# alexmeli100/pbrt-rust

Hardware: AMD Instinct MI355X
Metric: Msamples/s (camera rays x spp) at 1920x1080 (higher is better)
Workload: dtype f32

## Files before the change

### pbrt-rust_amd/csrc/dev_light.h

```cpp
#pragma once
#include "dev_scene.h"
#include "dev_sampler.h"
#include "dev_sphere.h"

namespace ptd {

PT_DEV int find_interval_cdf(const float *cdf, int size, float u) {
    int first = 0, len = size;
    while (len > 0) {
        int half = len >> 1, middle = first + half;
        if (cdf[middle] <= u) { first = middle + 1; len -= half + 1; }
        else len = half;
    }
    int r = first - 1;
    return r < 0 ? 0 : (r > size - 2 ? size - 2 : r);
}

struct Dist1D { const float *func; const float *cdf; float func_int; int n; };

PT_DEV int dist_sample_discrete(const Dist1D &d, float u, float &pdf) {
    if (d.n >= 1 && d.n <= 3) {
        const int n = d.n;
        const float c0 = d.cdf[0], c1 = d.cdf[1], c2 = d.cdf[n < 2 ? n : 2], c3 = d.cdf[n < 3 ? n : 3];
        const float f0 = d.func[0], f1 = d.func[n < 2 ? 0 : 1], f2 = d.func[n < 3 ? 0 : 2];
        int first = 0, len = n + 1;
        while (len > 0) {
            const int half = len >> 1, middle = first + half;
            const float cm = middle == 0 ? c0 : middle == 1 ? c1 : middle == 2 ? c2 : c3;
            if (cm <= u) { first = middle + 1; len -= half + 1; }
            else len = half;
        }
        const int r = first - 1;
        const int off = r < 0 ? 0 : (r > n - 1 ? n - 1 : r);
        const float fo = off == 0 ? f0 : off == 1 ? f1 : f2;
        pdf = (d.func_int > 0.0f) ? fo / (d.func_int * (float)n) : 0.0f;
        return off;
    }
    int off = find_interval_cdf(d.cdf, d.n + 1, u);
    pdf = (d.func_int > 0.0f) ? d.func[off] / (d.func_int * (float)d.n) : 0.0f;
    return off;
}
PT_DEV float dist_sample_continuous(const Dist1D &d, float u, float &pdf, int &off) {
    off = find_interval_cdf(d.cdf, d.n + 1, u);
    float du = u - d.cdf[off];
    float diff = d.cdf[off + 1] - d.cdf[off];
    if (diff > 0.0f) du /= diff;
    pdf = (d.func_int > 0.0f) ? d.func[off] / d.func_int : 0.0f;
    return ((float)off + du) / (float)d.n;
}

struct IData { V3 p, p_error, n; };

PT_DEV void spawn_ray(const IData &it, V3 d, V3 &o) { o = offset_ray_origin(it.p, it.p_error, it.n, d); }
PT_DEV void spawn_ray_to(const IData &a, const IData &b, V3 &o, V3 &d) {
    o = offset_ray_origin(a.p, a.p_error, a.n, b.p - a.p);
    V3 t = offset_ray_origin(b.p, b.p_error, b.n, o - b.p);
    d = t - o;
}

PT_DEV RGB env_lookup(const DeviceScene &s, P2 st) {
    int w = (int)s.env_w, h = (int)s.env_h;
    float sf = st.x * (float)w - 0.5f, tf = st.y * (float)h - 0.5f;
    int64_t s0 = f2i_sat(floorf(sf)), t0 = f2i_sat(floorf(tf));
    float ds = sf - (float)s0, dt = tf - (float)t0;
    auto wrap = [](int64_t v, int n) -> int {
        if (v >= -(int64_t)n && v < 2 * (int64_t)n) { int r = (int)v; if (r < 0) r += n; else if (r >= n) r -= n; return r; }
        int64_t r = v % n; if (r < 0) r += n;
        return (int)r;
    };
    const int sa = wrap(s0, w), sb = wrap(s0 + 1, w), ta = wrap(t0, h), tb = wrap(t0 + 1, h);
    auto texel = [&](int si, int ti) -> RGB {
        const float *p = s.env_texels + 3 * ((size_t)ti * w + si);
        return RGB(p[0], p[1], p[2]);
    };
    RGB tmp1 = texel(sb, tb) * (ds * dt);
    RGB tmp2 = texel(sb, ta) * (ds * (1.0f - dt));
    RGB tmp3 = texel(sa, tb) * ((1.0f - ds) * dt);
    RGB tmp4 = texel(sa, ta) * ((1.0f - ds) * (1.0f - dt));
    return tmp4 + tmp3 + tmp2 + tmp1;
}

PT_DEV bool light_is_delta(const PtLight &L) { return L.type == PT_LIGHT_DISTANT || L.type == PT_LIGHT_POINT || L.type == PT_LIGHT_SPOT; }

PT_DEV RGB area_l(const PtLight &L, V3 n, V3 w) {
    if (L.two_sided || dot(n, w) > 0.0f) return RGB(L.L[0], L.L[1], L.L[2]);
    return RGB(0.0f);
}
struct LightTri { V3 p0, p1, p2, n_sample, n_pdf; uint32_t fl, tri; float area, inv_area; RGB Lemit; bool two_sided, degenerate; };
PT_DEV bool load_light_tri(const DeviceScene &s, uint32_t li, LightTri &t, bool for_pdf) {
    const float4 *r = s.light_rec + 6 * (size_t)li;
    const float4 q0 = r[0], q1 = r[1], q2 = r[2];
    t.p0 = V3(q0.x, q0.y, q0.z); t.p1 = V3(q1.x, q1.y, q1.z); t.p2 = V3(q2.x, q2.y, q2.z);
    const uint32_t bits = __float_as_uint(q0.w);
    t.fl = bits & 0xffu; t.degenerate = (bits & 0x200u) != 0u; t.tri = __float_as_uint(q1.w); t.area = q2.w;
    if (for_pdf) { const float4 q5 = r[5]; t.n_pdf = V3(q5.x, q5.y, q5.z); }
    else {
        const float4 q3 = r[3], q4 = r[4];
        t.Lemit = RGB(q3.x, q3.y, q3.z); t.two_sided = __float_as_uint(q3.w) != 0u;
        t.n_sample = V3(q4.x, q4.y, q4.z); t.inv_area = q4.w;
    }
    return (bits & 0x100u) != 0u;
}
PT_DEV RGB area_l(const LightTri &t, V3 n, V3 w) { return (t.two_sided || dot(n, w) > 0.0f) ? t.Lemit : RGB(0.0f); }
PT_DEV M4 ldm4(const float *p) { M4 m; for (int i = 0; i < 16; ++i) m.m[i] = p[i]; return m; }

PT_DEV RGB light_le(const DeviceScene &s, const PtLight &L, V3 ray_d) {
    if (L.type != PT_LIGHT_INFINITE) return RGB(0.0f);
    V3 w = normalize(xf_vector(ldm4(L.world_to_light), ray_d));
    P2 st(spherical_phi(w) * kInv2Pi, spherical_theta(w) * kInvPi);
    return env_lookup(s, st);
}

PT_DEV P2 env_sample_continuous(const DeviceScene &s, P2 u, float &pdf) {
    int nu = 2 * (int)s.env_w, nv = 2 * (int)s.env_h;
    Dist1D marg{s.env_marg_func, s.env_marg_cdf, s.env_marg_int, nv};
    float pdf1, pdf0; int v, dummy;
    float d1 = dist_sample_continuous(marg, u.y, pdf1, v);
    Dist1D cond{s.env_func + (size_t)v * nu, s.env_cdf + (size_t)v * (nu + 1), s.env_func_int[v], nu};
    float d0 = dist_sample_continuous(cond, u.x, pdf0, dummy);
    pdf = pdf0 * pdf1;
    return P2(d0, d1);
}
PT_DEV float env_pdf(const DeviceScene &s, P2 p) {
    int nu = 2 * (int)s.env_w, nv = 2 * (int)s.env_h;
    uint32_t iu = f2u32_sat(p.x * (float)nu); if (iu > (uint32_t)(nu - 1)) iu = nu - 1;
    uint32_t iv = f2u32_sat(p.y * (float)nv); if (iv > (uint32_t)(nv - 1)) iv = nv - 1;
    return s.env_func[(size_t)iv * nu + iu] / s.env_marg_int;
}

PT_DEV IData sphere_sample_interaction(const PtSphere &S, const IData &ref, P2 u, float &pdf) {
    const M4 o2w = ldm4g(S.object_to_world), w2o = ldm4g(S.world_to_object);
    const V3 pcenter = xf_point(o2w, V3(0.0f, 0.0f, 0.0f));
    const V3 porigin = offset_ray_origin(ref.p, ref.p_error, ref.n, pcenter - ref.p);
    IData it;
    if (distance_squared(porigin, pcenter) <= S.radius * S.radius) {
        const float z = 1.0f - 2.0f * u.x;
        const float r = sqrtf(maxf(1.0f - z * z, 0.0f));
        const float phi = 2.0f * kPi * u.y;
        float sn, cs; dm_sincosf(phi, sn, cs);
        V3 pobj = V3(0.0f, 0.0f, 0.0f) + V3(r * cs, r * sn, z) * S.radius;
        it.n = normalize(xf_normal_inv(w2o, pobj));
        if (S.reverse_orientation) it.n = it.n * -1.0f;
        pobj = pobj * (S.radius / length(pobj));
        const V3 perr = vabs(pobj) * gammaf(5);
        it.p = xf_point_abs_err(o2w, pobj, perr, it.p_error);
        pdf = 1.0f / (S.phi_max * S.radius * (S.z_max - S.z_min));
        V3 wi = it.p - ref.p;
        if (length_squared(wi) == 0.0f) pdf = 0.0f;
        else { wi = normalize(wi); pdf *= distance_squared(ref.p, it.p) / abs_dot(it.n, -wi); }
        if (__builtin_isinf(pdf)) pdf = 0.0f;
        return it;
    }
    const float dc = length(ref.p - pcenter);
    const float invdc = 1.0f / dc;
    const V3 wc = (pcenter - ref.p) * invdc; V3 wcx, wcy;
    coordinate_system(wc, wcx, wcy);
    const float sin_thetamax = S.radius * invdc;
    const float sin_thetamax2 = sin_thetamax * sin_thetamax;
    const float inv_sin_thetamax = 1.0f / sin_thetamax;
    const float cos_thetamax = sqrtf(maxf(1.0f - sin_thetamax2, 0.0f));
    float cos_theta = (cos_thetamax - 1.0f) * u.x + 1.0f;
    float sin_theta2 = 1.0f - cos_theta * cos_theta;
    if (sin_thetamax2 < 0.00068523f) { sin_theta2 = sin_thetamax2 * u.x; cos_theta = sqrtf(1.0f - sin_theta2); }
    const float cos_alpha = sin_theta2 * inv_sin_thetamax + cos_theta * sqrtf(maxf(1.0f - sin_theta2 * inv_sin_thetamax * inv_sin_thetamax, 0.0f));
    const float sin_alpha = sqrtf(maxf(1.0f - cos_alpha * cos_alpha, 0.0f));
    const float phi = u.y * 2.0f * kPi;
    float sn, cs; dm_sincosf(phi, sn, cs);
    const V3 nworld = (-wcx) * sin_alpha * cs + (-wcy) * sin_alpha * sn + (-wc) * cos_alpha;
    const V3 pworld = pcenter + V3(nworld.x, nworld.y, nworld.z) * S.radius;
    it.p = pworld; it.p_error = vabs(pworld) * gammaf(5); it.n = V3(0.0f, 0.0f, 0.0f);
    pdf = 1.0f / (2.0f * kPi * (1.0f - cos_thetamax));
    return it;
}

template <bool SPH> PT_DEV RGB light_sample_li(const DeviceScene &s, uint32_t li, const IData &ref, P2 u, V3 &wi, float &pdf, IData &p1) {
    p1.p = V3(); p1.p_error = V3(); p1.n = V3();
    {
        LightTri t;
        if (load_light_tri(s, li, t, false)) {
            const float su0 = sqrtf(u.x);
            const float b0 = 1.0f - su0, b1 = u.y * su0;
            IData it;
            const float b2 = 1.0f - b0 - b1;
            it.p = t.p0 * b0 + t.p1 * b1 + t.p2 * b2;
            it.n = t.n_sample;
            if (t.fl & PT_TRI_HAS_N) {
                const uint32_t i0 = s.indices[3 * t.tri], i1 = s.indices[3 * t.tri + 1], i2 = s.indices[3 * t.tri + 2];
                const V3 ns = ld3(s.N, i0) * b0 + ld3(s.N, i1) * b1 + ld3(s.N, i2) * b2;
                it.n = face_forward(it.n, ns);
            }
            const V3 pabs = vabs(t.p0 * b0) + vabs(t.p1 * b1) + vabs(t.p2 * b2);
            it.p_error = pabs * gammaf(6);
            pdf = t.inv_area;
            V3 w = it.p - ref.p;
            if (length_squared(w) == 0.0f) pdf = 0.0f;
            else {
                w = normalize(w);
                pdf *= distance_squared(ref.p, it.p) / abs_dot(it.n, -w);
                if (__builtin_isinf(pdf)) pdf = 0.0f;
            }
            if (pdf == 0.0f || length_squared(it.p - ref.p) == 0.0f) { pdf = 0.0f; return RGB(0.0f); }
            wi = normalize(it.p - ref.p);
            p1 = it;
            return area_l(t, it.n, -wi);
        }
    }
    const PtLight &L = s.lights[li];
    switch (L.type) {
    case PT_LIGHT_DIFFUSE_AREA: {
        if (SPH && (s.prim_shape[L.prim] >> 30) == PT_SHAPE_SPHERE && s.spheres[s.prim_shape[L.prim] & 0x3fffffffu].kind == PT_QUADRIC_DISK) {
            const PtSphere &S = s.spheres[s.prim_shape[L.prim] & 0x3fffffffu];
            const P2 pd = concentric_sample_disk(u);
            const M4 o2w = ldm4g(S.object_to_world), w2o = ldm4g(S.world_to_object);
            IData it;
            it.n = normalize(xf_normal_inv(w2o, V3(0.0f, 0.0f, 0.1f)));
            if (S.reverse_orientation) it.n = it.n * -1.0f;
            it.p = xf_point_abs_err(o2w, V3(pd.x * S.radius, pd.y * S.radius, S.z_min), V3(0.0f, 0.0f, 0.0f), it.p_error);
            pdf = 1.0f / s.light_area[li];
            V3 w = it.p - ref.p;
            if (length_squared(w) == 0.0f) pdf = 0.0f;
            else {
                w = normalize(w);
                pdf *= distance_squared(ref.p, it.p) / abs_dot(it.n, -w);
                if (__builtin_isinf(pdf)) pdf = 0.0f;
            }
            if (pdf == 0.0f || length_squared(it.p - ref.p) == 0.0f) { pdf = 0.0f; return RGB(0.0f); }
            wi = normalize(it.p - ref.p);
            p1 = it;
            return area_l(L, it.n, -wi);
        }
        if (SPH && (s.prim_shape[L.prim] >> 30) == PT_SHAPE_SPHERE) {
            IData it = sphere_sample_interaction(s.spheres[s.prim_shape[L.prim] & 0x3fffffffu], ref, u, pdf);
            if (pdf == 0.0f || length_squared(it.p - ref.p) == 0.0f) { pdf = 0.0f; return RGB(0.0f); }
            wi = normalize(it.p - ref.p);
            p1 = it;
            return area_l(L, it.n, -wi);
        }
        pdf = 0.0f; return RGB(0.0f);
    }
    case PT_LIGHT_DISTANT: {
        V3 wl(L.dir[0], L.dir[1], L.dir[2]);
        wi = wl; pdf = 1.0f;
        p1.p = ref.p + wl * (2.0f * s.world_radius);
        return RGB(L.L[0], L.L[1], L.L[2]);
    }
    case PT_LIGHT_POINT: {
        V3 pl(L.pos[0], L.pos[1], L.pos[2]);
        wi = normalize(pl - ref.p); pdf = 1.0f;
        p1.p = pl;
        return RGB(L.L[0], L.L[1], L.L[2]) / distance_squared(pl, ref.p);
    }
    case PT_LIGHT_SPOT: {
        V3 pl(L.pos[0], L.pos[1], L.pos[2]);
        wi = normalize(pl - ref.p); pdf = 1.0f;
        p1.p = pl;
        V3 wl = normalize(xf_vector(ldm4(L.world_to_light), -wi));
        float cos_theta = wl.z, fall;
        if (cos_theta < L.cos_total_width) fall = 0.0f;
        else if (cos_theta >= L.cos_falloff_start) fall = 1.0f;
        else { float delta = (cos_theta - L.cos_total_width) / (L.cos_falloff_start - L.cos_total_width); fall = (delta * delta) * (delta * delta); }
        return RGB(L.L[0], L.L[1], L.L[2]) * fall / distance_squared(pl, ref.p);
    }
    case PT_LIGHT_INFINITE: {
        float map_pdf = 0.0f;
        P2 uv = env_sample_continuous(s, u, map_pdf);
        if (map_pdf == 0.0f) { pdf = 0.0f; return RGB(0.0f); }
        float theta = uv.y * kPi, phi = uv.x * 2.0f * kPi;
        float cos_t, sin_t, sin_p, cos_p;
        dm_sincosf(theta, sin_t, cos_t);
        dm_sincosf(phi, sin_p, cos_p);
        V3 v(sin_t * cos_p, sin_t * sin_p, cos_t);
        wi = xf_vector(ldm4(L.light_to_world), v);
        pdf = map_pdf / (2.0f * kPi * kPi * sin_t);
        if (sin_t == 0.0f) pdf = 0.0f;
        p1.p = ref.p + wi * (2.0f * s.world_radius);
        return env_lookup(s, uv);
    }
    default: pdf = 0.0f; return RGB(0.0f);
    }
}

template <bool SPH> PT_DEV float light_pdf_li(const DeviceScene &s, uint32_t li, const IData &ref, V3 wi) {
    {
        LightTri t;
        if (load_light_tri(s, li, t, true)) {
            V3 o; spawn_ray(ref, wi, o);
            float th, b0, b1, b2;
            if (!tri_hit_params(t.p0, t.p1, t.p2, o, wi, PT_INF, th, b0, b1, b2)) return 0.0f;
            if (t.degenerate) return 0.0f;
            const V3 ip = t.p0 * b0 + t.p1 * b1 + t.p2 * b2;
            const V3 in = t.n_pdf;
            float pdf = distance_squared(ref.p, ip) / (dot(in, -wi) * t.area);
            if (__builtin_isinf(pdf)) pdf = 0.0f;
            return pdf;
        }
    }
    const PtLight &L = s.lights[li];
    if (SPH && L.type == PT_LIGHT_DIFFUSE_AREA && (s.prim_shape[L.prim] >> 30) == PT_SHAPE_SPHERE && s.spheres[s.prim_shape[L.prim] & 0x3fffffffu].kind == PT_QUADRIC_DISK) {
        const PtSphere &S = s.spheres[s.prim_shape[L.prim] & 0x3fffffffu];
        V3 o; spawn_ray(ref, wi, o);
        SurfaceInteraction il;
        if (!sphere_fill_interaction(S, o, wi, il, false)) return 0.0f;
        float pdf = distance_squared(ref.p, il.p) / (dot(il.n, -wi) * s.light_area[li]);
        if (__builtin_isinf(pdf)) pdf = 0.0f;
        return pdf;
    }
    if (SPH && L.type == PT_LIGHT_DIFFUSE_AREA && (s.prim_shape[L.prim] >> 30) == PT_SHAPE_SPHERE) {
        const PtSphere &S = s.spheres[s.prim_shape[L.prim] & 0x3fffffffu];
        const V3 pcenter = xf_point(ldm4g(S.object_to_world), V3(0.0f, 0.0f, 0.0f));
        const V3 porigin = offset_ray_origin(ref.p, ref.p_error, ref.n, pcenter - ref.p);
        if (distance_squared(porigin, pcenter) <= S.radius * S.radius) {
            V3 o; spawn_ray(ref, wi, o);
            SurfaceInteraction il;
            if (!sphere_fill_interaction(S, o, wi, il)) return 0.0f;
            float pdf = distance_squared(ref.p, il.p) / (dot(il.n, -wi) * s.light_area[li]);
            if (__builtin_isinf(pdf)) pdf = 0.0f;
            return pdf;
        }
        const float sin_thetamax2 = S.radius * S.radius / distance_squared(ref.p, pcenter);
        const float cos_thetamax = sqrtf(maxf(1.0f - sin_thetamax2, 0.0f));
        return 1.0f / (2.0f * kPi * (1.0f - cos_thetamax));
    }
    if (L.type == PT_LIGHT_DIFFUSE_AREA) return 0.0f;
    if (L.type == PT_LIGHT_INFINITE) {
        V3 w = xf_vector(ldm4(L.world_to_light), wi);
        float theta = spherical_theta(w), phi = spherical_phi(w);
        float sin_t = dm_sinf(theta);
        if (sin_t == 0.0f) return 0.0f;
        return env_pdf(s, P2(phi * kInv2Pi, theta * kInvPi)) / (2.0f * kPi * kPi * sin_t);
    }
    return 0.0f;
}

struct LightGrid {
    int strategy;
    uint32_t nvox[3];
    uint32_t n_lights;
    const float *func;
    const float *cdf;
    const float *func_int;
    const unsigned long long *cell_ptr;
    unsigned long long zero_block;
    uint32_t *missing;
};
PT_DEV size_t light_grid_cell(const LightGrid &g, const DeviceScene &s, V3 p) {
    float o[3] = {p.x - s.wb_min[0], p.y - s.wb_min[1], p.z - s.wb_min[2]};
    uint32_t pi[3];
    for (int i = 0; i < 3; ++i) {
        if (s.wb_max[i] > s.wb_min[i]) o[i] /= s.wb_max[i] - s.wb_min[i];
        const float x = o[i] * (float)g.nvox[i];
        const uint32_t hi = g.nvox[i] - 1u;
        const uint32_t v = (x > 0.0f) ? (uint32_t)(int32_t)fminf(x, 2147483520.0f) : 0u;
        pi[i] = v > hi ? hi : v;
    }
    return ((size_t)pi[2] * g.nvox[1] + pi[1]) * g.nvox[0] + pi[0];
}
PT_DEV Dist1D light_distribution_lookup(const LightGrid &g, const DeviceScene &s, V3 p) {
    size_t cell = 0;
    if (g.strategy == PT_LS_SPATIAL) cell = light_grid_cell(g, s, p);
    if (g.cell_ptr) {
        const unsigned long long b = g.cell_ptr[cell];
        if (b == g.zero_block) atomicAdd(g.missing, 1u);
        const float *blk = reinterpret_cast<const float *>(b);
        Dist1D d{blk + 4, blk + 4 + g.n_lights, blk[0], (int)g.n_lights};
        return d;
    }
    Dist1D d{g.func + cell * g.n_lights, g.cdf + cell * (g.n_lights + 1), g.func_int[cell], (int)g.n_lights};
    return d;
}

}
```

### pbrt-rust_amd/csrc/dev_scene.h

```cpp
#pragma once
#include "dev_math.h"
#include "../../include/mi355pt.h"

namespace ptd {

struct TriPacket {
    float x[3]; uint32_t prim;
    float y[3]; uint32_t shape;
    float z[3]; uint32_t flags;
};
enum { TP_ALPHA = 1u << 7, TP_BOGUS = 1u << 8, TP_SPHERE = 1u << 9, TP_LAST = 1u << 10, TP_INSTANCE = 1u << 11 };
constexpr uint32_t kTpClassShift = 12, kTpClassMask = 15u, kTpMatShift = 16, kTpMatNone = 0xffffu;

struct WideNode {
    float lmin[3]; float lmax0;
    float lmax12[2]; float rmin01[2];
    float rmin2; float rmax[3];
    uint32_t left_ref, right_ref;
    uint32_t meta;
    uint32_t pad;
};
struct QuadNode {
    float lo[3][4];
    float hi[3][4];
    uint32_t ref[4];
    uint32_t meta; uint32_t pad[3];
};
static_assert(sizeof(QuadNode) == 128, "QuadNode is one 128-byte line");
constexpr uint32_t kLeafBit = 0x80000000u;
constexpr uint32_t kRefMask = 0x01ffffffu;
constexpr uint32_t kRefMaskQuad = 0x7fffffffu;

struct DevInstance {
    float world_to_instance[16], instance_to_world[16];
    float root_min[3], root_max[3];
    uint32_t root_ref;
    uint32_t single;
    uint32_t identity;
    uint32_t root_ref4;
};

struct DevGridAux { const float *density; float sigma_t, inv_max_density; };

struct DevBssTable { int n_rho, n_radius; const float *rho_samples, *radius_samples, *profile, *rhoeff, *profile_cdf; };

struct DevImage { uint32_t width, height, n_levels, channels; const float *texels; uint32_t level_offset[16]; };

struct DeviceScene {
    const WideNode *wide; uint32_t n_nodes;
    float root_min[3], root_max[3]; uint32_t root_ref;
    const QuadNode *quad; uint32_t root_ref4; uint32_t leaf_off, pool_quads;
    const TriPacket *leaf; uint32_t n_prims;
    const float *P; const float *N; const float *S; const float *UV;
    const uint32_t *indices; const uint8_t *tri_flags; uint32_t n_triangles;
    const PtSphere *spheres; uint32_t n_spheres;
    const DevInstance *instances; uint32_t n_instances;
    const uint32_t *prim_shape; const uint32_t *prim_material; const uint32_t *prim_light;
    const PtMaterial *materials; uint32_t n_materials;
    const PtLight *lights; uint32_t n_lights;
    const float *light_area;
    const float4 *light_rec;
    const uint32_t *infinite_lights; uint32_t n_infinite;
    const uint8_t *mat_class;
    const DevBssTable *bss_tables; uint32_t n_bss_tables;
    const PtMedium *media; uint32_t n_media;
    uint32_t has_shells;
    const DevGridAux *grid_aux; uint32_t has_grid;
    const uint32_t *prim_med_in; const uint32_t *prim_med_out;
    const PtTexture *textures; uint32_t n_textures; const uint32_t *tex_prog_offset; const uint32_t *tex_prog;
    const DevImage *images; const float *ewa_lut;
    const int32_t *tri_alpha; const int32_t *tri_shadow_alpha;
    uint32_t env_w, env_h; const float *env_texels;
    const float *env_func; const float *env_cdf; const float *env_func_int;
    const float *env_marg_func; const float *env_marg_cdf; float env_marg_int;
    float wb_min[3], wb_max[3];
    float world_radius; float world_center[3];
};

struct Ray { V3 o, d; float t_max; };

struct Hit { uint32_t prim; float t, b0, b1, b2; };

PT_DEV V3 ld3(const float *p, uint32_t i) { return V3(p[3 * i], p[3 * i + 1], p[3 * i + 2]); }

struct TriRay { int kz; float Sx, Sy, Sz; };
PT_DEV TriRay tri_ray_setup(V3 rd) {
    TriRay r;
    r.kz = max_dimension(vabs(rd));
    float dx, dy, dz;
    if (r.kz == 0) { dx = rd.y; dy = rd.z; dz = rd.x; }
    else if (r.kz == 1) { dx = rd.z; dy = rd.x; dz = rd.y; }
    else { dx = rd.x; dy = rd.y; dz = rd.z; }
    r.Sx = -dx / dz; r.Sy = -dy / dz; r.Sz = 1.0f / dz;
    return r;
}
PT_DEV V3 tri_permute(V3 v, int kz) { const bool k0 = kz == 0, k1 = kz == 1; return V3(k0 ? v.y : (k1 ? v.z : v.x), k0 ? v.z : (k1 ? v.x : v.y), k0 ? v.x : (k1 ? v.y : v.z)); }
PT_DEV uint32_t tp_aux(uint32_t w0, uint32_t w1, uint32_t w2, int kz, int axis) {
    const bool k0 = kz == 0, k1 = kz == 1;
    if (axis == 2) return k0 ? w1 : (k1 ? w0 : w2);
    if (axis == 1) return k0 ? w0 : (k1 ? w2 : w1);
    return k0 ? w2 : (k1 ? w1 : w0);
}
PT_DEV bool tri_hit_core(V3 p0t, V3 p1t, V3 p2t, const TriRay &tr, float t_max, float &t, float &b0, float &b1, float &b2) {
    const float Sx = tr.Sx, Sy = tr.Sy, Sz = tr.Sz;
    p0t.x += Sx * p0t.z; p0t.y += Sy * p0t.z;
    p1t.x += Sx * p1t.z; p1t.y += Sy * p1t.z;
    p2t.x += Sx * p2t.z; p2t.y += Sy * p2t.z;
    float e0 = p1t.x * p2t.y - p1t.y * p2t.x;
    float e1 = p2t.x * p0t.y - p2t.y * p0t.x;
    float e2 = p0t.x * p1t.y - p0t.y * p1t.x;
    if (e0 == 0.0f || e1 == 0.0f || e2 == 0.0f) {
        double p2txp1ty = (double)p2t.x * (double)p1t.y, p2typ1tx = (double)p2t.y * (double)p1t.x;
        e0 = (float)(p2typ1tx - p2txp1ty);
        double p0txp2ty = (double)p0t.x * (double)p2t.y, p0typ2tx = (double)p0t.y * (double)p2t.x;
        e1 = (float)(p0typ2tx - p0txp2ty);
        double p1txp0ty = (double)p1t.x * (double)p0t.y, p1typ0tx = (double)p1t.y * (double)p0t.x;
        e2 = (float)(p1typ0tx - p1txp0ty);
    }
    const bool mixed = ((e0 < 0.0f) | (e1 < 0.0f) | (e2 < 0.0f)) & ((e0 > 0.0f) | (e1 > 0.0f) | (e2 > 0.0f));
    float det = e0 + e1 + e2;
    p0t.z *= Sz; p1t.z *= Sz; p2t.z *= Sz;
    float tscaled = e0 * p0t.z + e1 * p1t.z + e2 * p2t.z;
    const float tmd = t_max * det;
    const bool out_neg = (det < 0.0f) & ((tscaled >= 0.0f) | (tscaled < tmd));
    const bool out_pos = (det > 0.0f) & ((tscaled <= 0.0f) | (tscaled >= tmd));
    if (mixed | (det == 0.0f) | out_neg | out_pos) return false;
    float invdet = 1.0f / det;
    b0 = e0 * invdet; b1 = e1 * invdet; b2 = e2 * invdet;
    t = tscaled * invdet;
    float maxzt = max_component(vabs(V3(p0t.z, p1t.z, p2t.z)));
    float deltaz = gammaf(3) * maxzt;
    float maxxt = max_component(vabs(V3(p0t.x, p1t.x, p2t.x)));
    float maxyt = max_component(vabs(V3(p0t.y, p1t.y, p2t.y)));
    float deltax = gammaf(5) * (maxxt + maxzt);
    float deltay = gammaf(5) * (maxyt + maxzt);
    float deltae = 2.0f * (gammaf(2) * maxxt * maxyt + deltay * maxxt + deltax * maxyt);
    float maxe = max_component(vabs(V3(e0, e1, e2)));
    float deltat = 3.0f * (gammaf(3) * maxe * maxzt + deltae * maxzt + deltaz * maxe) * fabsf(invdet);
    if (t <= deltat) return false;
    return true;
}
PT_DEV bool tri_hit_params(V3 p0, V3 p1, V3 p2, V3 ro, const TriRay &tr, float t_max, float &t, float &b0, float &b1, float &b2) {
    return tri_hit_core(tri_permute(p0 - ro, tr.kz), tri_permute(p1 - ro, tr.kz), tri_permute(p2 - ro, tr.kz), tr, t_max, t, b0, b1, b2);
}

PT_DEV bool tri_hit_params(V3 p0, V3 p1, V3 p2, V3 ro, V3 rd, float t_max, float &t, float &b0, float &b1, float &b2) {
    return tri_hit_params(p0, p1, p2, ro, tri_ray_setup(rd), t_max, t, b0, b1, b2);
}

PT_DEV void tri_uvs(const DeviceScene &s, uint32_t tri, uint32_t i0, uint32_t i1, uint32_t i2, P2 uv[3]) {
    if (s.tri_flags[tri] & PT_TRI_HAS_UV) {
        uv[0] = P2(s.UV[2 * i0], s.UV[2 * i0 + 1]); uv[1] = P2(s.UV[2 * i1], s.UV[2 * i1 + 1]); uv[2] = P2(s.UV[2 * i2], s.UV[2 * i2 + 1]);
    } else { uv[0] = P2(0.0f, 0.0f); uv[1] = P2(1.0f, 0.0f); uv[2] = P2(1.0f, 1.0f); }
}
PT_DEV bool tri_partials(V3 p0, V3 p1, V3 p2, const P2 uv[3], V3 &dpdu, V3 &dpdv) {
    float duv02x = uv[0].x - uv[2].x, duv02y = uv[0].y - uv[2].y;
    float duv12x = uv[1].x - uv[2].x, duv12y = uv[1].y - uv[2].y;
    V3 dp02 = p0 - p2, dp12 = p1 - p2;
    float determinant = duv02x * duv12y - duv02y * duv12x;
    bool degenerateuv = fabsf(determinant) < 1.0e-8f;
    dpdu = V3(); dpdv = V3();
    if (!degenerateuv) {
        float invdet = 1.0f / determinant;
        dpdu = (dp02 * duv12y - dp12 * duv02y) * invdet;
        dpdv = (dp02 * -duv12x + dp12 * duv02x) * invdet;
    }
    if (degenerateuv || length_squared(cross(dpdu, dpdv)) == 0.0f) {
        V3 ng = cross(p2 - p0, p1 - p0);
        if (length_squared(ng) == 0.0f) return false;
        coordinate_system(normalize(ng), dpdu, dpdv);
    }
    return true;
}

struct SurfaceInteraction {
    V3 p, p_error, n, wo;
    V3 dpdu;
    V3 sh_n, sh_dpdu;
    V3 dpdv; P2 uv;
    V3 sh_dpdv, sh_dndu, sh_dndv;
    bool has_shape, shape_flip;
    uint32_t prim;
};
PT_DEV void tri_fill_from(const DeviceScene &s, uint32_t tri, uint32_t fl, V3 p0, V3 p1, V3 p2, V3 ray_d, float b0, float b1, float b2, bool with_shape, SurfaceInteraction &si) {
    uint32_t i0 = 0, i1 = 0, i2 = 0;
    if (fl & (PT_TRI_HAS_N | PT_TRI_HAS_S | PT_TRI_HAS_UV)) { i0 = s.indices[3 * tri]; i1 = s.indices[3 * tri + 1]; i2 = s.indices[3 * tri + 2]; }
    P2 uv[3];
    if (fl & PT_TRI_HAS_UV) { uv[0] = P2(s.UV[2 * i0], s.UV[2 * i0 + 1]); uv[1] = P2(s.UV[2 * i1], s.UV[2 * i1 + 1]); uv[2] = P2(s.UV[2 * i2], s.UV[2 * i2 + 1]); }
    else { uv[0] = P2(0.0f, 0.0f); uv[1] = P2(1.0f, 0.0f); uv[2] = P2(1.0f, 1.0f); }
    V3 dpdu, dpdv; tri_partials(p0, p1, p2, uv, dpdu, dpdv);
    V3 dp02 = p0 - p2, dp12 = p1 - p2;
    float xabs = fabsf(b0 * p0.x) + fabsf(b1 * p1.x) + fabsf(b2 * p2.x);
    float yabs = fabsf(b0 * p0.y) + fabsf(b1 * p1.y) + fabsf(b2 * p2.y);
    float zabs = fabsf(b0 * p0.z) + fabsf(b1 * p1.z) + fabsf(b2 * p2.z);
    si.p_error = V3(xabs, yabs, zabs) * gammaf(7);
    si.p = p0 * b0 + p1 * b1 + p2 * b2;
    si.dpdu = dpdu; si.sh_dpdu = dpdu; si.dpdv = dpdv; si.sh_dpdv = dpdv;
    si.sh_dndu = V3(0.0f, 0.0f, 0.0f); si.sh_dndv = V3(0.0f, 0.0f, 0.0f);
    si.uv = P2(uv[0].x * b0 + uv[1].x * b1 + uv[2].x * b2, uv[0].y * b0 + uv[1].y * b1 + uv[2].y * b2);
    bool flip = ((fl & PT_TRI_REVERSE_ORIENTATION) != 0) != ((fl & PT_TRI_SWAPS_HANDEDNESS) != 0);
    si.has_shape = with_shape; si.shape_flip = flip;
    V3 nn = normalize(cross(dp02, dp12));
    si.n = nn; si.sh_n = nn;
    si.wo = -ray_d;
    if (flip) { si.n = -nn; si.sh_n = -nn; }
    if (fl & (PT_TRI_HAS_N | PT_TRI_HAS_S)) {
        V3 ns;
        if (fl & PT_TRI_HAS_N) {
            ns = ld3(s.N, i0) * b0 + ld3(s.N, i1) * b1 + ld3(s.N, i2) * b2;
            if (length_squared(ns) > 0.0f) ns = normalize(ns); else ns = si.n;
        } else ns = si.n;
        V3 ss;
        if (fl & PT_TRI_HAS_S) {
            ss = ld3(s.S, i0) * b0 + ld3(s.S, i1) * b1 + ld3(s.S, i2) * b2;
            if (length_squared(ss) > 0.0f) ss = normalize(ss); else ss = normalize(si.dpdu);
        } else ss = normalize(si.dpdu);
        V3 ts = cross(ss, ns);
        if (length_squared(ts) > 0.0f) { ts = normalize(ts); ss = cross(ts, ns); }
        else coordinate_system(ns, ss, ts);
        if (fl & PT_TRI_HAS_N) {
            const float duv02x = uv[0].x - uv[2].x, duv02y = uv[0].y - uv[2].y, duv12x = uv[1].x - uv[2].x, duv12y = uv[1].y - uv[2].y;
            const V3 n0 = ld3(s.N, i0), n1 = ld3(s.N, i1), n2 = ld3(s.N, i2);
            const V3 dn1 = n0 - n2, dn2 = n1 - n2;
            const float det = duv02x * duv12y - duv02y * duv12x;
            if (fabsf(det) < 1.0e-8f) {
                const V3 dn = cross(n2 - n0, n1 - n0);
                if (length_squared(dn) != 0.0f) coordinate_system(dn, si.sh_dndu, si.sh_dndv);
            } else {
                const float invdet = 1.0f / det;
                si.sh_dndu = (dn1 * duv12y - dn2 * duv02y) * invdet;
                si.sh_dndv = (dn1 * -duv12x + dn2 * duv02x) * invdet;
            }
        }
        if (fl & PT_TRI_REVERSE_ORIENTATION) ts = -ts;
        si.sh_n = normalize(cross(ss, ts));
        if (with_shape) {
            if (flip) si.sh_n = -si.sh_n;
            si.n = face_forward(si.n, si.sh_n);
        }
        si.sh_dpdu = ss; si.sh_dpdv = ts;
    }
}
PT_DEV void tri_fill_interaction(const DeviceScene &s, uint32_t tri, V3 ray_d, float b0, float b1, float b2, bool with_shape, SurfaceInteraction &si) {
    const uint32_t i0 = s.indices[3 * tri], i1 = s.indices[3 * tri + 1], i2 = s.indices[3 * tri + 2];
    tri_fill_from(s, tri, s.tri_flags[tri], ld3(s.P, i0), ld3(s.P, i1), ld3(s.P, i2), ray_d, b0, b1, b2, with_shape, si);
}
PT_DEV float tri_area(V3 p0, V3 p1, V3 p2) { return 0.5f * length(cross(p1 - p0, p2 - p0)); }

PT_DEV bool slab_test(const float bmin[3], const float bmax[3], V3 ro, V3 inv_dir, bool nx, bool ny, bool nz, float ray_tmax) {
    float tmin = ((nx ? bmax[0] : bmin[0]) - ro.x) * inv_dir.x;
    float tmax = ((nx ? bmin[0] : bmax[0]) - ro.x) * inv_dir.x;
    float tymin = ((ny ? bmax[1] : bmin[1]) - ro.y) * inv_dir.y;
    float tymax = ((ny ? bmin[1] : bmax[1]) - ro.y) * inv_dir.y;
    const float k = 1.0f + 2.0f * gammaf(3);
    tmax *= k; tymax *= k;
    if (tmin > tymax || tymin > tmax) return false;
    if (tymin > tmin) tmin = tymin;
    if (tymax < tmax) tmax = tymax;
    float tzmin = ((nz ? bmax[2] : bmin[2]) - ro.z) * inv_dir.z;
    float tzmax = ((nz ? bmin[2] : bmax[2]) - ro.z) * inv_dir.z;
    tzmax *= k;
    if (tmin > tzmax || tzmin > tmax) return false;
    if (tzmin > tmin) tmin = tzmin;
    if (tzmax < tmax) tmax = tzmax;
    return (tmin < ray_tmax) && (tmax > 0.0f);
}
PT_DEV bool slab_geo(const float bmin[3], const float bmax[3], V3 ro, V3 inv_dir, bool nx, bool ny, bool nz, float &tmin_out) {
    float tmin = ((nx ? bmax[0] : bmin[0]) - ro.x) * inv_dir.x;
    float tmax = ((nx ? bmin[0] : bmax[0]) - ro.x) * inv_dir.x;
    const float tymin = ((ny ? bmax[1] : bmin[1]) - ro.y) * inv_dir.y;
    float tymax = ((ny ? bmin[1] : bmax[1]) - ro.y) * inv_dir.y;
    const float tzmin = ((nz ? bmax[2] : bmin[2]) - ro.z) * inv_dir.z;
    float tzmax = ((nz ? bmin[2] : bmax[2]) - ro.z) * inv_dir.z;
    const float k = 1.0f + 2.0f * gammaf(3);
    tmax *= k; tymax *= k; tzmax *= k;
    const bool miss_xy = (tmin > tymax) | (tymin > tmax);
    tmin = (tymin > tmin) ? tymin : tmin;
    tmax = (tymax < tmax) ? tymax : tmax;
    const bool miss_z = (tmin > tzmax) | (tzmin > tmax);
    tmin = (tzmin > tmin) ? tzmin : tmin;
    tmax = (tzmax < tmax) ? tzmax : tmax;
    tmin_out = tmin;
    return !(miss_xy | miss_z) & (tmax > 0.0f);
}

}
```

### pbrt-rust_amd/csrc/kern_decl.h

```cpp
#pragma once
#include "kern_common.h"

template <int ANY, int MODE, bool PROBE, int QUADK> __global__ void k_trace(DeviceScene s, TraceJob job);
template <int MAXL, int MODE, int DIFF> __global__ void k_shade(DeviceScene s, RenderConst rc, SobolTables tabs, LightGrid grid, PathSoA ps, ShadeJob job);
template <bool SPH, bool VOL> __global__ void k_shade_miss(DeviceScene s, RenderConst rc, PathSoA ps, ShadeJob job);
template <bool SPH, bool VOL> __global__ void k_bssrdf(DeviceScene s, RenderConst rc, SobolTables tabs, LightGrid grid, PathSoA ps, BssrdfJob job);
__global__ void k_medium_route(DeviceScene s, RenderConst rc, SobolTables tabs, PathSoA ps, const uint32_t *queue, const uint32_t *count_ptr,
                               uint32_t *class_count, uint32_t *c0, uint32_t *c1, uint32_t *c2, uint32_t *c3, uint32_t *c4, uint32_t *c5, uint32_t *error);
__global__ void k_shade_medium(DeviceScene s, RenderConst rc, SobolTables tabs, LightGrid grid, PathSoA ps, ShadeJob job);
__global__ void k_build_packets(DeviceScene s, const uint32_t *ordered, uint32_t n_refs, TriPacket *out);
__global__ void k_mark_leaf_ends(TriPacket *leaf, const uint32_t *last_index, uint32_t n);
__global__ void k_light_area(DeviceScene s, float *area, float4 *rec);
template <int NQ, int CAP> __global__ void k_route(DeviceScene s, const uint32_t *queue, const uint32_t *count_ptr, PathSoA ps, uint32_t *class_count, RouteJob rj);
__global__ void k_generate(RenderConst rc, SobolTables tabs, PathSoA ps, uint32_t *q_ext, uint32_t *q_ext_count, DevCounters *counters);
__global__ void k_film(RenderConst rc, PathSoA ps, const float *filter_table, float *film_rgbw, DevCounters *counters);
template <bool SPH> __global__ void k_film_final(DeviceScene s, RenderConst rc, PathSoA ps, const float *filter_table, float *film_rgbw, DevCounters *counters);
__global__ void k_film_finish(const float *film_rgbw, float *film_xyzw, uint32_t npix);
__global__ void k_film_resolve(const float4 *film_xyzw, uint32_t n_pixels, float scale, float *rgb, uint8_t *srgb8, int packed);
__global__ void k_film_halves_error(const float4 *film_a, const float4 *film_b, uint32_t width, uint32_t height, uint32_t ntx, float *tile_sum, float *tile_err);
__global__ void k_film_error_reduce(const float *tile_sum, const float *tile_err, uint32_t n_tiles, float n_pixels, float *out);
__global__ void k_tiles_select(RenderConst rc, const float *tile_err, float threshold, const uint32_t *candidates, uint32_t n_candidates, uint32_t *out);
__global__ void k_film_sum(FilmSumArgs a, float4 *dst, int accumulate, size_t n_quads);
__global__ void k_light_grid_contrib(DeviceScene s, uint32_t nvx, uint32_t nvy, uint32_t nvz, float *func, const uint32_t *cells, size_t n_cells, size_t stride);
__global__ void k_light_grid_finish(uint32_t n_lights, size_t ncell, float *func, float *cdf, float *func_int, const uint32_t *cells, size_t stride, unsigned long long *cell_ptr);
template <bool SPH> __global__ void k_light_touch(DeviceScene s, LightGrid g, PathSoA ps, const uint32_t *queue, const uint32_t *count_ptr, uint32_t kind, uint32_t max_depth, uint32_t *req_flag, uint32_t *req_list, uint32_t *req_count);
__global__ void k_halton_samples(SobolTables tabs, HaltonParams hp, uint32_t n, const int32_t *pixel_xy, const uint32_t *sample_num,
                                 uint32_t n_dims, float *out, uint64_t *out_index);
__global__ void k_sobol_samples(SobolTables tabs, SobolParams sp, uint32_t n, const int32_t *pixel_xy, const uint32_t *sample_num,
                                uint32_t n_dims, float *out, uint64_t *out_index);
__global__ void k_camera_rays(RenderConst rc, uint32_t n, const float *cs, float *out_o, float *out_d);
__global__ void k_dist1d_sample(const float *func, const float *cdf, float func_int, int n, int discrete, uint32_t n_u, const float *u, float *out_x, float *out_pdf, int32_t *out_off);
```

### pbrt-rust_amd/csrc/kern_misc.h

```cpp
#pragma once
#include "kern_common.h"
#include "kern_film.h"
__global__ void k_build_packets(DeviceScene s, const uint32_t *ordered, uint32_t n_refs, TriPacket *out) {
    uint32_t i = blockIdx.x * blockDim.x + threadIdx.x;
    if (i >= n_refs) return;
    uint32_t prim = ordered[i];
    TriPacket p;
    if (prim & PT_TOP_INSTANCE) {
        p.x[0] = p.x[1] = p.x[2] = p.y[0] = p.y[1] = p.y[2] = p.z[0] = p.z[1] = p.z[2] = 0.0f;
        p.prim = PT_NONE; p.shape = prim & ~PT_TOP_INSTANCE; p.flags = TP_INSTANCE;
        out[i] = p;
        return;
    }
    uint32_t shape = s.prim_shape[prim];
    p.prim = prim; p.shape = shape; p.flags = 0;
    const uint32_t mat = s.prim_material[prim];
    const uint32_t hi = ((mat == PT_NONE ? 0u : (uint32_t)s.mat_class[mat]) << kTpClassShift) | ((mat == PT_NONE || mat >= kTpMatNone ? kTpMatNone : mat) << kTpMatShift);
    if ((shape >> 30) == PT_SHAPE_TRIANGLE) {
        uint32_t tri = shape & 0x3fffffffu;
        uint32_t i0 = s.indices[3 * tri], i1 = s.indices[3 * tri + 1], i2 = s.indices[3 * tri + 2];
        V3 p0 = ld3(s.P, i0), p1 = ld3(s.P, i1), p2 = ld3(s.P, i2);
        P2 uv[3]; tri_uvs(s, tri, i0, i1, i2, uv);
        V3 dpdu, dpdv;
        bool ok = tri_partials(p0, p1, p2, uv, dpdu, dpdv);
        p.x[0] = p0.x; p.x[1] = p1.x; p.x[2] = p2.x; p.y[0] = p0.y; p.y[1] = p1.y; p.y[2] = p2.y; p.z[0] = p0.z; p.z[1] = p1.z; p.z[2] = p2.z;
        p.flags = (uint32_t)s.tri_flags[tri] | (ok ? 0u : (uint32_t)TP_BOGUS) | hi;
        if ((s.tri_alpha && s.tri_alpha[tri] >= 0) || (s.tri_shadow_alpha && s.tri_shadow_alpha[tri] >= 0)) p.flags |= TP_ALPHA;
    } else {
        p.x[0] = p.x[1] = p.x[2] = p.y[0] = p.y[1] = p.y[2] = p.z[0] = p.z[1] = p.z[2] = 0.0f;
        p.flags = TP_SPHERE | hi;
    }
    out[i] = p;
}

__global__ void k_mark_leaf_ends(TriPacket *leaf, const uint32_t *last_index, uint32_t n) {
    uint32_t i = blockIdx.x * blockDim.x + threadIdx.x;
    if (i < n) leaf[last_index[i]].flags |= TP_LAST;
}

__global__ void k_light_area(DeviceScene s, float *area, float4 *rec) {
    uint32_t i = blockIdx.x * blockDim.x + threadIdx.x;
    if (i >= s.n_lights) return;
    float a = 0.0f;
    const PtLight &L = s.lights[i];
    float4 r0 = make_float4(0.0f, 0.0f, 0.0f, 0.0f), r1 = r0, r2 = r0, r4 = r0, r5 = r0;
    if (L.type == PT_LIGHT_DIFFUSE_AREA) {
        uint32_t shape = s.prim_shape[L.prim];
        if ((shape >> 30) == PT_SHAPE_TRIANGLE) {
            uint32_t tri = shape & 0x3fffffffu;
            const V3 p0 = ld3(s.P, s.indices[3 * tri]), p1 = ld3(s.P, s.indices[3 * tri + 1]), p2 = ld3(s.P, s.indices[3 * tri + 2]);
            a = tri_area(p0, p1, p2);
            const uint32_t fl = s.tri_flags[tri];
            const bool flip = ((fl & PT_TRI_REVERSE_ORIENTATION) != 0) != ((fl & PT_TRI_SWAPS_HANDEDNESS) != 0);
            V3 ns = normalize(cross(p1 - p0, p2 - p0));
            if (!(fl & PT_TRI_HAS_N) && flip) ns = ns * -1.0f;
            V3 np = normalize(cross(p0 - p2, p1 - p2));
            if (flip) np = -np;
            P2 uv[3]; tri_uvs(s, tri, s.indices[3 * tri], s.indices[3 * tri + 1], s.indices[3 * tri + 2], uv);
            V3 dpdu, dpdv;
            const bool degenerate = !tri_partials(p0, p1, p2, uv, dpdu, dpdv);
            r4 = make_float4(ns.x, ns.y, ns.z, 1.0f / a); r5 = make_float4(np.x, np.y, np.z, 0.0f);
            r0 = make_float4(p0.x, p0.y, p0.z, __uint_as_float(fl | 0x100u | (degenerate ? 0x200u : 0u)));
            r1 = make_float4(p1.x, p1.y, p1.z, __uint_as_float(tri)); r2 = make_float4(p2.x, p2.y, p2.z, a);
        } else {
            const PtSphere &S = s.spheres[shape & 0x3fffffffu];
            a = S.kind == PT_QUADRIC_DISK ? S.phi_max * 0.5f * (S.radius * S.radius - S.inner_radius * S.inner_radius)
                                          : S.phi_max * S.radius * (S.z_max - S.z_min);
        }
    }
    area[i] = a;
    float4 *r = rec + 6 * (size_t)i;
    r[0] = r0; r[1] = r1; r[2] = r2; r[3] = make_float4(L.L[0], L.L[1], L.L[2], __uint_as_float(L.two_sided)); r[4] = r4; r[5] = r5;
}
template <int NQ, int CAP>
__global__ __launch_bounds__(256) void k_route(DeviceScene s, const uint32_t *queue, const uint32_t *count_ptr, PathSoA ps, uint32_t *class_count, RouteJob rj) {
    __shared__ LdsQueue<CAP> q[NQ];
#pragma unroll
    for (int k = 0; k < NQ; ++k) lq_init(q[k]);
    __syncthreads();
    const uint32_t count = *count_ptr;
    const uint32_t rounded = (count + 255u) & ~255u;
    for (uint32_t qi = blockIdx.x * blockDim.x + threadIdx.x; qi < rounded; qi += gridDim.x * blockDim.x) {
        const bool valid = qi < count;
        uint32_t pid = 0, cls = (uint32_t)kMissClass;
        if (valid) {
            pid = queue[qi];
            cls = (ps.hit_pflags(pid) >> kTpClassShift) & kTpClassMask;
        }
        const uint32_t slot = (uint32_t)(rj.slot_map >> (4u * cls)) & 15u;
        if (valid && slot == 15u && cls != rj.drop_cls) atomicMax(rj.error, (uint32_t)PT_ERR_UNSUPPORTED);
#pragma unroll
        for (int k = 0; k < NQ; ++k) if ((uint32_t)k < rj.n_slots) lq_push(q[k], pid, valid && slot == (uint32_t)k);
        __syncthreads();
#pragma unroll
        for (int k = 0; k < NQ; ++k) if ((uint32_t)k < rj.n_slots) lq_flush_nosync(q[k], class_count + rj.cls_of_slot[k], rj.buf[k], 256u, false);
        __syncthreads();
    }
#pragma unroll
    for (int k = 0; k < NQ; ++k) if ((uint32_t)k < rj.n_slots) lq_flush_nosync(q[k], class_count + rj.cls_of_slot[k], rj.buf[k], 0u, true);
}
PT_DEV void camera_ray(const RenderConst &rc, float pfx, float pfy, float time_u, P2 plens_u, V3 &o, V3 &d) {
    V3 pcamera = xf_point(rc.raster_to_camera, V3(pfx, pfy, 0.0f));
    V3 ro(0.0f, 0.0f, 0.0f), rd = normalize(pcamera);
    if (rc.lens_radius > 0.0f) {
        P2 dsk = concentric_sample_disk(plens_u);
        float lx = dsk.x * rc.lens_radius, ly = dsk.y * rc.lens_radius;
        float ft = rc.focal_distance / rd.z;
        V3 pfocus = ro + rd * ft;
        ro = V3(lx, ly, 0.0f);
        rd = normalize(pfocus - ro);
    }
    (void)time_u;
    V3 oerr;
    V3 ow = xf_point_err(rc.camera_to_world, ro, oerr);
    V3 dw = xf_vector(rc.camera_to_world, rd);
    float l2 = length_squared(dw);
    if (l2 > 0.0f) { float dt = dot(vabs(dw), oerr) / l2; ow = ow + dw * dt; }
    o = ow; d = dw;
}

constexpr int kGenPlane = 257;
struct GenStage { float4 core[4 * kGenPlane]; float4 ray[2 * kGenPlane]; uint32_t alive[256]; };
PT_DEV void stage_path(GenStage &g, uint32_t t, float pfx, float pfy, V3 o, V3 d, uint64_t index, uint32_t medium) {
    g.core[0 * kGenPlane + t] = make_float4(0.0f, 0.0f, 0.0f, 1.0f);
    g.core[1 * kGenPlane + t] = make_float4(1.0f, 1.0f, 1.0f, __uint_as_float(5u | (PF_CAMERA_RAY << 24)));
    g.core[2 * kGenPlane + t] = make_float4(__uint_as_float((uint32_t)index), __uint_as_float((uint32_t)(index >> 32)), pfx, pfy);
    g.core[3 * kGenPlane + t] = make_float4(__uint_as_float(medium), __uint_as_float(PT_NONE), 0.0f, 0.0f);
    g.ray[0 * kGenPlane + t] = make_float4(o.x, o.y, o.z, d.x); g.ray[1 * kGenPlane + t] = make_float4(d.y, d.z, 0.0f, 0.0f);
}
PT_DEV void flush_paths(const GenStage &g, const PathSoA &ps, uint32_t pid0, uint32_t t) {
    float4 *core = reinterpret_cast<float4 *>(ps.core) + 4 * (size_t)pid0, *ray = reinterpret_cast<float4 *>(ps.ray) + 2 * (size_t)pid0;
#pragma unroll
    for (uint32_t j = 0; j < 4; ++j) { const uint32_t gq = j * 256u + t, p = gq >> 2, q = gq & 3u; if (g.alive[p]) core[gq] = g.core[q * kGenPlane + p]; }
#pragma unroll
    for (uint32_t j = 0; j < 2; ++j) { const uint32_t gq = j * 256u + t, p = gq >> 1, q = gq & 1u; if (g.alive[p]) ray[gq] = g.ray[q * kGenPlane + p]; }
}

__global__ __launch_bounds__(256) void k_generate(RenderConst rc, SobolTables tabs, PathSoA ps, uint32_t *q_ext, uint32_t *q_ext_count, DevCounters *counters) {
    constexpr uint32_t kVdcNibbles = 13;
    __shared__ uint32_t s_nib[kSobolNibbles * 5 * 16];
    __shared__ uint64_t s_vdc[2 * kVdcNibbles * 16];
    __shared__ LdsQueue<1024> s_q;
    __shared__ GenStage s_gen;
    lq_init(s_q);
    const uint32_t m = (uint32_t)rc.sobol.log2_resolution;
    sobol_stage_lds(s_nib, tabs.nib, 5u, threadIdx.x, blockDim.x);
    if (m > 0) for (uint32_t i = threadIdx.x; i < 2 * kVdcNibbles * 16; i += blockDim.x) {
        const uint32_t which = i / (kVdcNibbles * 16), e = i - which * (kVdcNibbles * 16), j = e >> 4, n = e & 15u;
        const uint64_t *col = (which ? tabs.vdc_inv : tabs.vdc) + (m - 1) * 52 + 4 * j;
        uint64_t v = 0;
        for (uint32_t b = 0; b < 4; ++b) if (n & (1u << b)) v ^= col[b];
        s_vdc[i] = v;
    }
    __syncthreads();
    const uint32_t total = rc.n_pix_slots * rc.s_count;
    const uint32_t stride = gridDim.x * blockDim.x;
    const uint32_t rounded = (total + 255u) & ~255u;
    unsigned long long n_alive = 0;
    for (uint32_t pid = blockIdx.x * blockDim.x + threadIdx.x; pid < rounded; pid += stride) {
        bool alive = false;
        if (pid < total) {
            const uint32_t slot = pid % rc.n_pix_slots, sl = pid / rc.n_pix_slots;
            int32_t px, py;
            if (slot_to_pixel(rc, slot, px, py)) {
                const uint64_t sample = rc.s_begin + sl;
                if (rc.halton.enabled) {
                    const uint64_t index = halton_index_for_sample(rc.halton, px, py, sample);
                    const float fx = halton_sample_dimension(tabs, rc.halton, index, 0u), fy = halton_sample_dimension(tabs, rc.halton, index, 1u);
                    const float pfx = (float)px + fx, pfy = (float)py + fy;
                    const float tm = halton_sample_dimension(tabs, rc.halton, index, 2u);
                    const P2 pl(halton_sample_dimension(tabs, rc.halton, index, 3u), halton_sample_dimension(tabs, rc.halton, index, 4u));
                    V3 o, d;
                    camera_ray(rc, pfx, pfy, tm, pl, o, d);
                    stage_path(s_gen, threadIdx.x, pfx, pfy, o, d, index, rc.volpath ? rc.camera_medium : PT_NONE);
                    alive = true;
                } else {
                uint64_t index = 0;
                if (m != 0) {
                    index = sample << (m << 1);
                    uint64_t delta = 0;
                    for (uint64_t f = sample, j = 0; f != 0; f >>= 4, ++j) delta ^= s_vdc[j * 16 + (f & 15u)];
                    uint64_t b = ((uint64_t)((uint32_t)(px - rc.sobol.sb_min[0]) << m) | (uint64_t)(uint32_t)(py - rc.sobol.sb_min[1])) ^ delta;
                    for (uint32_t j = 0; b != 0; b >>= 4, ++j) index ^= s_vdc[kVdcNibbles * 16 + j * 16 + (b & 15u)];
                }
                const uint32_t v0 = sobol_bits_nib(s_nib, 5u * 16u, tabs.m32, index), v1 = sobol_bits_nib(s_nib + 16, 5u * 16u, tabs.m32 + 52, index), v2 = sobol_bits_nib(s_nib + 32, 5u * 16u, tabs.m32 + 104, index),
                               v3 = sobol_bits_nib(s_nib + 48, 5u * 16u, tabs.m32 + 156, index), v4 = sobol_bits_nib(s_nib + 64, 5u * 16u, tabs.m32 + 208, index);
                float fx = sobol_to_float(v0) * (float)rc.sobol.resolution + (float)rc.sobol.sb_min[0];
                fx = clampf(fx - (float)px, 0.0f, kOneMinusEps);
                float fy = sobol_to_float(v1) * (float)rc.sobol.resolution + (float)rc.sobol.sb_min[1];
                fy = clampf(fy - (float)py, 0.0f, kOneMinusEps);
                const float pfx = (float)px + fx, pfy = (float)py + fy;
                V3 o, d;
                camera_ray(rc, pfx, pfy, sobol_to_float(v2), P2(sobol_to_float(v3), sobol_to_float(v4)), o, d);
                stage_path(s_gen, threadIdx.x, pfx, pfy, o, d, index, rc.volpath ? rc.camera_medium : PT_NONE);
                alive = true;
                }
            }
        }
        s_gen.alive[threadIdx.x] = alive ? 1u : 0u;
        __syncthreads();
        flush_paths(s_gen, ps, pid - threadIdx.x, threadIdx.x);
        lq_push(s_q, pid, alive);
        lq_sync_flush(s_q, q_ext_count, q_ext, 256u, false);
        n_alive += alive ? 1ull : 0ull;
    }
    lq_sync_flush(s_q, q_ext_count, q_ext, 0u, true);
    counter_add(&counters->camera_rays, n_alive);
}
__global__ __launch_bounds__(256) void k_film(RenderConst rc, PathSoA ps, const float *filter_table, float *film_rgbw, DevCounters *counters) {
    film_slot(rc, ps, filter_table, film_rgbw, counters, [](uint32_t, RGB &) {});
}

__global__ void k_film_finish(const float *film_rgbw, float *film_xyzw, uint32_t npix) {
    uint32_t i = blockIdx.x * blockDim.x + threadIdx.x;
    if (i >= npix) return;
    float rgb[3] = {film_rgbw[4 * i], film_rgbw[4 * i + 1], film_rgbw[4 * i + 2]}, xyz[3];
    rgb_to_xyz(rgb, xyz);
    film_xyzw[4 * i] += xyz[0]; film_xyzw[4 * i + 1] += xyz[1]; film_xyzw[4 * i + 2] += xyz[2]; film_xyzw[4 * i + 3] += film_rgbw[4 * i + 3];
}
__global__ void k_film_sum(FilmSumArgs a, float4 *dst, int accumulate, size_t n_quads) {
    const size_t i = (size_t)blockIdx.x * blockDim.x + threadIdx.x;
    if (i >= n_quads) return;
    float4 s = a.src[0][i];
    for (uint32_t k = 1; k < a.n; ++k) { const float4 b = a.src[k][i]; s = make_float4(s.x + b.x, s.y + b.y, s.z + b.z, s.w + b.w); }
    if (accumulate) { const float4 d = dst[i]; s = make_float4(d.x + s.x, d.y + s.y, d.z + s.z, d.w + s.w); }
    dst[i] = s;
}

__global__ __launch_bounds__(256) void k_light_grid_contrib(DeviceScene s, uint32_t nvx, uint32_t nvy, uint32_t nvz, float *func, const uint32_t *cells, size_t n_cells, size_t stride) {
    const size_t gid = (size_t)blockIdx.x * blockDim.x + threadIdx.x;
    const size_t ncell = cells ? n_cells : (size_t)nvx * nvy * nvz;
    if (gid >= ncell * s.n_lights) return;
    const uint32_t j = (uint32_t)(gid % s.n_lights);
    const size_t slot = gid / s.n_lights;
    const size_t cell = cells ? (size_t)cells[slot] : slot;
    const uint32_t pi0 = (uint32_t)(cell % nvx), pi1 = (uint32_t)((cell / nvx) % nvy), pi2 = (uint32_t)(cell / ((size_t)nvx * nvy));
    V3 p0((float)pi0 / (float)nvx, (float)pi1 / (float)nvy, (float)pi2 / (float)nvz);
    V3 p1((float)(pi0 + 1) / (float)nvx, (float)(pi1 + 1) / (float)nvy, (float)(pi2 + 1) / (float)nvz);
    V3 a(lerpf(p0.x, s.wb_min[0], s.wb_max[0]), lerpf(p0.y, s.wb_min[1], s.wb_max[1]), lerpf(p0.z, s.wb_min[2], s.wb_max[2]));
    V3 b(lerpf(p1.x, s.wb_min[0], s.wb_max[0]), lerpf(p1.y, s.wb_min[1], s.wb_max[1]), lerpf(p1.z, s.wb_min[2], s.wb_max[2]));
    V3 vmin(minf(a.x, b.x), minf(a.y, b.y), minf(a.z, b.z)), vmax(maxf(a.x, b.x), maxf(a.y, b.y), maxf(a.z, b.z));
    float contrib = 0.0f;
    for (uint32_t i = 0; i < 128; ++i) {
        V3 u3(radical_inverse(0, i), radical_inverse(1, i), radical_inverse(2, i));
        IData intr;
        intr.p = V3(lerpf(u3.x, vmin.x, vmax.x), lerpf(u3.y, vmin.y, vmax.y), lerpf(u3.z, vmin.z, vmax.z));
        P2 u(radical_inverse(3, i), radical_inverse(4, i));
        float pdf = 0.0f; V3 wi; IData vis;
        RGB Li = light_sample_li<true>(s, j, intr, u, wi, pdf, vis);
        if (pdf > 0.0f) contrib += Li.y() / pdf;
    }
    func[cells ? slot * stride + 4 + j : gid] = contrib;
}
__global__ __launch_bounds__(256) void k_light_grid_finish(uint32_t n_lights, size_t ncell, float *func, float *cdf, float *func_int, const uint32_t *cells, size_t stride, unsigned long long *cell_ptr) {
    const size_t cell = (size_t)blockIdx.x * blockDim.x + threadIdx.x;
    if (cell >= ncell) return;
    float *f = cells ? func + cell * stride + 4 : func + cell * n_lights, *c = cells ? f + n_lights : cdf + cell * (n_lights + 1);
    float sum = 0.0f;
    for (uint32_t j = 0; j < n_lights; ++j) sum += f[j];
    const float avg = sum / (128.0f * (float)n_lights);
    const float min_contrib = (avg > 0.0f) ? 0.001f * avg : 1.0f;
    for (uint32_t j = 0; j < n_lights; ++j) f[j] = maxf(f[j], min_contrib);
    c[0] = 0.0f;
    for (uint32_t i = 1; i < n_lights + 1; ++i) c[i] = c[i - 1] + f[i - 1] / (float)n_lights;
    const float fi = c[n_lights];
    if (fi == 0.0f) { for (uint32_t i = 1; i < n_lights + 1; ++i) c[i] = (float)i / (float)n_lights; }
    else { for (uint32_t i = 1; i < n_lights + 1; ++i) c[i] /= fi; }
    if (cells) { func[cell * stride] = fi; __threadfence(); cell_ptr[cells[cell]] = (unsigned long long)(func + cell * stride); }
    else func_int[cell] = fi;
}

template <bool SPH>
__global__ __launch_bounds__(256) void k_light_touch(DeviceScene s, LightGrid g, PathSoA ps, const uint32_t *queue, const uint32_t *count_ptr, uint32_t kind, uint32_t max_depth,
                                                     uint32_t *req_flag, uint32_t *req_list, uint32_t *req_count) {
    const uint32_t count = *count_ptr;
    for (uint32_t qi = blockIdx.x * blockDim.x + threadIdx.x; qi < count; qi += gridDim.x * blockDim.x) {
        const uint32_t pid = queue[qi];
        const uint32_t meta = ps.meta(pid);
        if ((meta >> 24) & PF_DEAD) continue;
        if (kind != 2u && ((meta >> 16) & 0xffu) >= max_depth) continue;
        const V3 ro(ps.ox(pid), ps.oy(pid), ps.oz(pid)), rd(ps.dx(pid), ps.dy(pid), ps.dz(pid));
        V3 p;
        if (kind == 1u) p = ro + rd * ps.hit_t(pid);
        else {
            if (ps.hit_prim(pid) == PT_NONE) continue;
            SurfaceInteraction si;
            fill_hit_pkt<SPH>(s, ps.hit_pkt(pid), SPH ? ps.hit_inst(pid) : PT_NONE, ro, rd, ps.hit_b0(pid), ps.hit_b1(pid), ps.hit_b2(pid), si);
            p = si.p;
        }
        const size_t cell = light_grid_cell(g, s, p);
        if (g.cell_ptr[cell] == g.zero_block && atomicExch(&req_flag[cell], 1u) == 0u) req_list[atomicAdd(req_count, 1u)] = (uint32_t)cell;
    }
}
__global__ void k_halton_samples(SobolTables tabs, HaltonParams hp, uint32_t n, const int32_t *pixel_xy, const uint32_t *sample_num,
                                 uint32_t n_dims, float *out, uint64_t *out_index) {
    uint32_t i = blockIdx.x * blockDim.x + threadIdx.x;
    if (i >= n) return;
    const uint64_t index = halton_index_for_sample(hp, pixel_xy[2 * i], pixel_xy[2 * i + 1], sample_num[i]);
    if (out_index) out_index[i] = index;
    for (uint32_t d = 0; d < n_dims; ++d) out[(size_t)i * n_dims + d] = halton_sample_dimension(tabs, hp, index, d);
}

__global__ __launch_bounds__(256) void k_sobol_samples(SobolTables tabs, SobolParams sp, uint32_t n, const int32_t *pixel_xy, const uint32_t *sample_num,
                                                       uint32_t n_dims, float *out, uint64_t *out_index) {
    constexpr uint32_t LDS_DIMS = 56u;
    __shared__ uint32_t s_sobol[LDS_DIMS * kSobolNibWords];
    sobol_stage_lds(s_sobol, tabs.nib, LDS_DIMS, threadIdx.x, blockDim.x);
    __syncthreads();
    uint32_t i = blockIdx.x * blockDim.x + threadIdx.x;
    if (i >= n) return;
    int32_t px = pixel_xy[2 * i], py = pixel_xy[2 * i + 1];
    uint64_t index = sobol_interval_to_index(tabs, (uint32_t)sp.log2_resolution, sample_num[i], (uint32_t)(px - sp.sb_min[0]), (uint32_t)(py - sp.sb_min[1]));
    if (out_index) out_index[i] = index;
    for (uint32_t d = 0; d < 2 && d < n_dims; ++d) out[(size_t)i * n_dims + d] = sobol_pixel_dim(tabs.m32, sp, index, (int)d, d == 0 ? px : py);
    Sampler smp; smp.index = index; smp.m32 = tabs.m32; smp.nib = tabs.nib; smp.lds = s_sobol; smp.lds_dims = LDS_DIMS; smp.overflow = false; smp.halton = false;
    smp.prime = tabs.prime; smp.prime_sum = tabs.prime_sum; smp.perm = tabs.perm;
    for (uint32_t d = 2; d < n_dims;) {
        smp.dim = d;
        smp.load_window();
        for (uint32_t k = 0; k < 8 && d < n_dims; ++k, ++d) out[(size_t)i * n_dims + d] = smp.get_1d();
    }
}
__global__ void k_camera_rays(RenderConst rc, uint32_t n, const float *cs, float *out_o, float *out_d) {
    uint32_t i = blockIdx.x * blockDim.x + threadIdx.x;
    if (i >= n) return;
    V3 o, d;
    camera_ray(rc, cs[5 * i], cs[5 * i + 1], cs[5 * i + 2], P2(cs[5 * i + 3], cs[5 * i + 4]), o, d);
    out_o[3 * i] = o.x; out_o[3 * i + 1] = o.y; out_o[3 * i + 2] = o.z;
    out_d[3 * i] = d.x; out_d[3 * i + 1] = d.y; out_d[3 * i + 2] = d.z;
}
__global__ void k_dist1d_sample(const float *func, const float *cdf, float func_int, int n, int discrete, uint32_t n_u, const float *u, float *out_x, float *out_pdf, int32_t *out_off) {
    uint32_t i = blockIdx.x * blockDim.x + threadIdx.x;
    if (i >= n_u) return;
    Dist1D d{func, cdf, func_int, n};
    float pdf = 0.0f; int off = 0; float x = 0.0f;
    if (discrete) off = dist_sample_discrete(d, u[i], pdf);
    else x = dist_sample_continuous(d, u[i], pdf, off);
    out_x[i] = x; out_pdf[i] = pdf; out_off[i] = off;
}
```

### pbrt-rust_amd/csrc/kern_shade_common.h

```cpp
#pragma once
#include "kern_common.h"

#ifdef PT_REGION_PROFILE
struct Prof { long long *t; int *r; unsigned long long *acc; };
#define PT_PROF_BEGIN __shared__ long long s_pt[4]; __shared__ int s_pr[4]; __shared__ unsigned long long s_pacc[64]; \
    if (threadIdx.x < 64) s_pacc[threadIdx.x] = 0; \
    if (threadIdx.x < 4) { s_pt[threadIdx.x] = clock64(); s_pr[threadIdx.x] = 15; } \
    Prof prof{s_pt, s_pr, s_pacc};
#define PT_PROF_END(counters) do { PT_T(14); __syncthreads(); \
    if (threadIdx.x < 16) atomicAdd(&(counters)->regions[threadIdx.x], prof.acc[threadIdx.x] + prof.acc[16 + threadIdx.x] + prof.acc[32 + threadIdx.x] + prof.acc[48 + threadIdx.x]); } while (0)
#define PT_T(k) do { if ((int)__lane_id() == __ffsll((unsigned long long)__ballot(1)) - 1) { const long long _n = clock64(); const int _w = threadIdx.x >> 6; \
    prof.acc[_w * 16 + prof.r[_w]] += (unsigned long long)(_n - prof.t[_w]); prof.t[_w] = _n; prof.r[_w] = (k); } } while (0)
#define PT_PROF_ARG , Prof prof
#define PT_PROF_PASS , prof
#else
#define PT_T(k) do {} while (0)
#define PT_PROF_BEGIN
#define PT_PROF_END(counters) do {} while (0)
#define PT_PROF_ARG
#define PT_PROF_PASS
#endif

template <bool SPH, bool VOL = false, bool EARLY = false> PT_DEV void resolve_pending(const DeviceScene &s, const PathSoA &ps, uint32_t pid, uint32_t &flags, RGB &L,
                                                unsigned long long &zero_num, uint32_t &n_assert, unsigned long long &n_bytes PT_PROF_ARG, Sampler *smp = nullptr) {
    if (!(flags & (PF_PEND_SHADOW | PF_PEND_MIS))) return;
    PT_T(1);
    const float4 *nq = reinterpret_cast<const float4 *>(ps.nee) + 4 * (size_t)pid;
    const float4 n1 = nq[1], n2 = nq[2], n3 = nq[3];
    float4 e0 = make_float4(0.0f, 0.0f, 0.0f, 0.0f), e1 = e0, e2 = e0, e3 = e0;
    if constexpr (EARLY) {
        if (flags & PF_PEND_MIS) { const float4 *mq = reinterpret_cast<const float4 *>(ps.mis) + 4 * (size_t)pid; e0 = mq[0]; e1 = mq[1]; e2 = mq[2]; e3 = mq[3]; }
        asm volatile("" :: "v"(n1.x), "v"(n2.x), "v"(n3.x), "v"(e0.x), "v"(e1.x), "v"(e2.x), "v"(e3.x));
    }
    n_bytes += 48 + ((flags & PF_PEND_MIS) ? 64 : 0);
    RGB Ld(0.0f);
    const uint32_t li = __float_as_uint(n1.w);
    if ((flags & PF_PEND_SHADOW) && (VOL ? __float_as_uint(n1.z) == PT_NONE : __float_as_uint(n1.z) == 0u)) {
        RGB A(n2.x, n2.y, n2.z);
        if (VOL) {
            const uint32_t sm = __float_as_uint(n3.w);
            if (sm != PT_NONE && s.media[sm].type == PT_MEDIUM_GRID) {
                const float4 n0 = nq[0];
                if (smp) A = A * grid_tr(s.media[sm], s.grid_aux[sm], V3(n0.x, n0.y, n0.z), V3(n0.w, n1.x, n1.y), 1.0f - kShadowEps, *smp);
                else A = RGB(0.0f);
            }
        }
        Ld = Ld + A;
    }
    if (flags & PF_PEND_MIS) {
        const float4 *mq = reinterpret_cast<const float4 *>(ps.mis) + 4 * (size_t)pid;
        const float4 m0 = EARLY ? e0 : mq[0], m1 = EARLY ? e1 : mq[1], m2 = EARLY ? e2 : mq[2], m3 = EARLY ? e3 : mq[3];
        const PtLight &Lt = s.lights[li];
        V3 wi(m0.w, m1.x, m1.y);
        RGB lrad(0.0f);
        const uint32_t mp = __float_as_uint(m2.x);
        if (mp != PT_NONE) {
            if (s.prim_light[mp] == li) {
                SurfaceInteraction lsi;
                fill_hit<SPH>(s, mp, PT_NONE, V3(m0.x, m0.y, m0.z), wi, m2.y, m2.z, m2.w, lsi);
                lrad = area_l(Lt, lsi.n, -wi);
            }
        } else { PT_T(2); lrad = light_le(s, Lt, wi); PT_T(1); }
        RGB Tr(1.0f);
        bool tr_done = false;
        if (VOL) {
            const uint32_t mm = ps.mis_medium(pid);
            if (mm != PT_NONE && s.media[mm].type == PT_MEDIUM_GRID) {
                Tr = smp ? RGB(grid_tr(s.media[mm], s.grid_aux[mm], V3(m0.x, m0.y, m0.z), wi, mp != PT_NONE ? m3.w : PT_INF, *smp)) : RGB(0.0f);
                tr_done = true;
            }
        }
        if (!lrad.is_black()) {
            RGB f(m3.x, m3.y, m3.z);
            if (VOL && !tr_done) {
                const uint32_t mm = ps.mis_medium(pid);
                if (mm != PT_NONE) Tr = Tr * medium_tr(s.media[mm], mp != PT_NONE ? m3.w : PT_INF, wi);
            }
            Ld = Ld + f * lrad * Tr * m1.z / m1.w;
        }
    }
    RGB nb(n3.x, n3.y, n3.z);
    RGB Ldb = nb * (Ld / n2.w);
    if (!VOL && Ldb.is_black() && !(flags & PF_NEE_UNCOUNTED)) zero_num++;
    if (!VOL && !(flags & PF_NEE_UNCOUNTED) && !(Ldb.y() >= 0.0f)) n_assert++;
    L = L + Ldb;
    flags &= ~(PF_PEND_SHADOW | PF_PEND_MIS | PF_NEE_UNCOUNTED);
}

template <bool SPH> PT_DEV bool vol_chain_step(const DeviceScene &s, const PathSoA &ps, uint32_t pid, uint32_t flags, Sampler &smp, bool &push_shadow, bool &push_mis,
                                              unsigned long long &n_bytes) {
    float4 *nq = reinterpret_cast<float4 *>(ps.nee) + 4 * (size_t)pid;
    float4 *mq = reinterpret_cast<float4 *>(ps.mis) + 4 * (size_t)pid;
    float4 *xq = reinterpret_cast<float4 *>(ps.ext) + 8 * (size_t)pid;
    if ((flags & PF_PEND_SHADOW) && __float_as_uint(nq[1].z) != 1u) {
        const float4 n0 = nq[0], n1 = nq[1], n2 = nq[2], n3 = nq[3], h0 = xq[4], h1 = xq[5];
        n_bytes += 64 + 32;
        const uint32_t prim = __float_as_uint(h0.x), sm = __float_as_uint(n3.w);
        const bool hit = prim != PT_NONE;
        const V3 so(n0.x, n0.y, n0.z), sd(n0.w, n1.x, n1.y);
        RGB A(n2.x, n2.y, n2.z);
        bool ended = true;
        if (hit && s.prim_material[prim] != PT_NONE) A = RGB(0.0f);
        else {
            if (sm != PT_NONE) {
                const float t_seg = hit ? h1.y : 1.0f - kShadowEps;
                A = A * (s.media[sm].type == PT_MEDIUM_GRID ? RGB(grid_tr(s.media[sm], s.grid_aux[sm], so, sd, t_seg, smp)) : medium_tr(s.media[sm], t_seg, sd));
            }
            if (hit) {
                SurfaceInteraction hs;
                fill_hit_pkt<SPH>(s, __float_as_uint(h1.z), SPH ? __float_as_uint(h1.x) : PT_NONE, so, sd, h0.y, h0.z, h0.w, hs);
                IData a; a.p = hs.p; a.p_error = hs.p_error; a.n = hs.n;
                IData b; { const float4 x0 = xq[0], x1 = xq[1], x2 = xq[2]; b.p = V3(x0.x, x0.y, x0.z); b.p_error = V3(x1.x, x1.y, x1.z); b.n = V3(x2.x, x2.y, x2.z); }
                V3 o2, d2; spawn_ray_to(a, b, o2, d2);
                const uint32_t sm2 = medium_toward(surface_iface(s, prim, sm), hs.n, d2);
                nq[0] = make_float4(o2.x, o2.y, o2.z, d2.x); nq[1] = make_float4(d2.y, d2.z, 0.0f, n1.w); nq[3] = make_float4(n3.x, n3.y, n3.z, __uint_as_float(sm2));
                push_shadow = true; ended = false; n_bytes += 48 + 4;
            }
        }
        nq[2] = make_float4(A.r, A.g, A.b, n2.w);
        if (!ended) return true;
        nq[1] = make_float4(n1.x, n1.y, __uint_as_float(1u), n1.w);
    }
    if (flags & PF_PEND_MIS) {
        const float4 m0 = mq[0], m1 = mq[1], m3 = mq[3], h0 = xq[6], h1 = xq[7];
        n_bytes += 64 + 32;
        const uint32_t prim = __float_as_uint(h0.x), mm = ps.mis_medium(pid);
        const bool hit = prim != PT_NONE;
        const V3 mo(m0.x, m0.y, m0.z), wi(m0.w, m1.x, m1.y);
        RGB f(m3.x, m3.y, m3.z);
        if (mm != PT_NONE) f = f * (s.media[mm].type == PT_MEDIUM_GRID ? RGB(grid_tr(s.media[mm], s.grid_aux[mm], mo, wi, hit ? h1.y : PT_INF, smp)) : medium_tr(s.media[mm], hit ? h1.y : PT_INF, wi));
        if (hit && s.prim_material[prim] == PT_NONE) {
            SurfaceInteraction hs;
            fill_hit_pkt<SPH>(s, __float_as_uint(h1.z), SPH ? __float_as_uint(h1.x) : PT_NONE, mo, wi, h0.y, h0.z, h0.w, hs);
            IData a; a.p = hs.p; a.p_error = hs.p_error; a.n = hs.n;
            V3 o2; spawn_ray(a, wi, o2);
            ps.mis_medium(pid) = medium_toward(surface_iface(s, prim, mm), hs.n, wi);
            mq[0] = make_float4(o2.x, o2.y, o2.z, wi.x); mq[3] = make_float4(f.r, f.g, f.b, m3.w);
            push_mis = true; n_bytes += 32 + 4;
            return true;
        }
        mq[2] = h0; mq[3] = make_float4(f.r, f.g, f.b, hit ? h1.y : 0.0f);
        ps.mis_medium(pid) = PT_NONE;
    }
    if (flags & PF_PEND_SHADOW) {
        const float4 n1 = nq[1], n3 = nq[3];
        nq[1] = make_float4(n1.x, n1.y, __uint_as_float(PT_NONE), n1.w); nq[3] = make_float4(n3.x, n3.y, n3.z, __uint_as_float(PT_NONE));
    }
    return false;
}


template <int QCAP, bool PROBE, bool SELF> struct VertexQueues {
    LdsQueue<QCAP> ext, res, sh, mis;
    LdsQueue<PROBE ? QCAP : 1> probe;
    LdsQueue<SELF ? QCAP : 1> self;
    PT_DEV void init() { lq_init(ext); lq_init(res); lq_init(sh); lq_init(mis); lq_init(probe); lq_init(self); }
    template <class Job> PT_DEV void push(const Job &job, uint32_t pid, bool to_ext, bool to_resolve, bool to_shadow, bool to_mis, bool to_self = false, bool to_probe = false) {
        lq_push(ext, pid, to_ext);
        lq_push(res, pid, to_resolve && job.shade_next0 != nullptr);
        lq_push(sh, pid, to_shadow);
        lq_push(mis, pid, to_mis);
        if constexpr (PROBE) if (job.probe_next) lq_push(probe, pid, to_probe);
        if constexpr (SELF) lq_push(self, pid, to_self);
    }
    template <class Job> PT_DEV void flush(const Job &job, uint32_t reserve, bool force) {
        __syncthreads();
        lq_flush_nosync(ext, job.ext_next_count, job.ext_next, reserve, force);
        lq_flush_nosync(res, job.shade_next0_count, job.shade_next0, reserve, force);
        lq_flush_nosync(sh, job.shadow_count, job.shadow, reserve, force);
        lq_flush_nosync(mis, job.mis_count, job.mis, reserve, force);
        if constexpr (PROBE) if (job.probe_next) lq_flush_nosync(probe, job.probe_next_count, job.probe_next, reserve, force);
        if constexpr (SELF) lq_flush_nosync(self, job.self_next_count, job.self_next, reserve, force);
        __syncthreads();
    }
};

PT_DEV bool russian_roulette(const RenderConst &rc, Sampler &smp, RGB &beta, float etascale, uint32_t bounces, uint32_t &n_assert) {
    const RGB rrbeta = beta * etascale;
    if (rrbeta.max_component_value() < rc.rr_threshold && bounces > 3) {
        const float q = maxf(1.0f - rrbeta.max_component_value(), 0.05f);
        if (smp.get_1d() < q) return true;
        beta = beta / (1.0f - q); if (__builtin_isinf(beta.y())) n_assert++;
    }
    return false;
}

PT_DEV uint32_t vertex_meta(const Sampler &smp, uint32_t bounces, uint32_t flags, uint32_t *error) {
    if (smp.overflow) atomicMax(error, (uint32_t)PT_ERR_SOBOL_DIMENSIONS);
    return (smp.dim & 0xffffu) | ((bounces & 0xffu) << 16) | (flags << 24);
}
PT_DEV void store_vertex(const PathSoA &ps, uint32_t pid, RGB L, RGB beta, const Sampler &smp, uint32_t bounces, uint32_t flags, uint32_t *error) {
    const uint32_t meta = vertex_meta(smp, bounces, flags, error);
    ps.L_r(pid) = L.r; ps.L_g(pid) = L.g; ps.L_b(pid) = L.b;
    ps.beta_r(pid) = beta.r; ps.beta_g(pid) = beta.g; ps.beta_b(pid) = beta.b;
    ps.meta(pid) = meta;
}

PT_DEV void add_escaped_le(const DeviceScene &s, V3 rd, RGB beta, RGB &L) {
    for (uint32_t k = 0; k < s.n_infinite; ++k) L = L + light_le(s, s.lights[s.infinite_lights[k]], rd) * beta;
}

PT_DEV void hist_init(uint32_t *s_hist) { if (threadIdx.x < 16) s_hist[threadIdx.x] = 0; }
PT_DEV void hist_add(uint32_t *s_hist, uint32_t bounces) { atomicAdd(&s_hist[bounces > 15u ? 15u : bounces], 1u); }
PT_DEV void vertex_epilogue(const uint32_t *s_hist, DevCounters *c, unsigned long long *items, unsigned long long *bytes, unsigned long long n_valid, unsigned long long n_bytes,
                            uint32_t n_assert) {
    if (threadIdx.x < 16 && s_hist[threadIdx.x]) atomicAdd(&c->path_len[threadIdx.x], (unsigned long long)s_hist[threadIdx.x]);
    counter_add(&c->ref_asserts, (unsigned long long)n_assert);
    counter_add(&c->stages, n_valid);
    counter_add(items, n_valid);
    counter_add(bytes, n_bytes);
}

template <bool SPH, class B, bool VOL = false, bool MEDIUM = false>
PT_DEV bool nee_vertex(const DeviceScene &s, const LightGrid &grid, const PathSoA &ps, uint32_t pid, Sampler &smp,
                                          const SurfaceInteraction &si, const IData &it, const B &bsdf, RGB beta, uint32_t &flags,
                                          bool &push_shadow, bool &push_mis, unsigned long long &n_bytes PT_PROF_ARG, MedIface mif = MedIface{PT_NONE, PT_NONE}) {
    bool nee_pending = false;
    if (s.n_lights > 0) {
        PT_T(5);
        Dist1D distrib = light_distribution_lookup(grid, s, si.p);
        float choice_pdf = 0.0f;
        const uint32_t li = (uint32_t)dist_sample_discrete(distrib, smp.get_1d(), choice_pdf);
        if (choice_pdf != 0.0f) {
            const P2 ulight = smp.get_2d();
            const P2 uscatt = smp.get_2d();
            const int bf = BSDF_ALL & ~BSDF_SPECULAR;
            V3 wi; float lightpdf = 0.0f, scattpdf = 0.0f; IData p1;
            RGB A(0.0f); V3 sh_o(0.0f, 0.0f, 0.0f), sh_d(0.0f, 0.0f, 0.0f);
            uint32_t sh_medium = PT_NONE;
            PT_T(6);
            RGB Li = light_sample_li<SPH>(s, li, it, ulight, wi, lightpdf, p1);
            PT_T(7);
            const bool delta = light_is_delta(s.lights[li]);
            if (lightpdf > 0.0f && !Li.is_black()) {
                RGB f = bsdf.f_pdf(si.wo, wi, bf, scattpdf);
                if (!MEDIUM) f = f * abs_dot(wi, si.sh_n);
                if (!f.is_black()) {
                    V3 so, sd; spawn_ray_to(it, p1, so, sd);
                    if (VOL) {
                        const uint32_t sm = medium_toward(mif, it.n, sd);
                        if (s.has_shells) {
                            sh_medium = sm;
                            float4 *xq = reinterpret_cast<float4 *>(ps.ext) + 8 * (size_t)pid;
                            xq[0] = make_float4(p1.p.x, p1.p.y, p1.p.z, 0.0f); xq[1] = make_float4(p1.p_error.x, p1.p_error.y, p1.p_error.z, 0.0f); xq[2] = make_float4(p1.n.x, p1.n.y, p1.n.z, 0.0f);
                            n_bytes += 48;
                        }
                        else if (sm != PT_NONE && s.media[sm].type == PT_MEDIUM_GRID) sh_medium = sm;
                        else if (sm != PT_NONE) Li = Li * medium_tr(s.media[sm], 1.0f - kShadowEps, sd);
                    }
                    A = delta ? f * Li / lightpdf : f * Li * power_heuristic(lightpdf, scattpdf) / lightpdf;
                    sh_o = so; sh_d = sd;
                    flags |= PF_PEND_SHADOW; push_shadow = true; nee_pending = true; n_bytes += 16 + 4;
                }
            }
            if (!delta) {
                PT_T(8);
                int sampled_type = 0;
                RGB f = bsdf.sample_f(si.wo, wi, uscatt, scattpdf, bf, sampled_type);
                if (!MEDIUM) f = f * abs_dot(wi, si.sh_n);
                const bool sampled_specular = (sampled_type & BSDF_SPECULAR) != 0;
                if (!f.is_black() && scattpdf > 0.0f) {
                    float weight = 1.0f;
                    bool skip = false;
                    if (!sampled_specular) {
                        PT_T(9);
                        lightpdf = light_pdf_li<SPH>(s, li, it, wi);
                        PT_T(8);
                        if (lightpdf == 0.0f) skip = true;
                        else weight = power_heuristic(scattpdf, lightpdf);
                    }
                    if (!skip) {
                        V3 mo; spawn_ray(it, wi, mo);
                        float4 *mq = reinterpret_cast<float4 *>(ps.mis) + 4 * (size_t)pid;
                        mq[0] = make_float4(mo.x, mo.y, mo.z, wi.x); mq[1] = make_float4(wi.y, wi.z, weight, scattpdf); mq[3] = make_float4(f.r, f.g, f.b, 0.0f);
                        if (VOL) ps.mis_medium(pid) = medium_toward(mif, it.n, wi);
                        flags |= PF_PEND_MIS; push_mis = true; nee_pending = true; n_bytes += 48 + 4;
                    }
                }
            }
            if (nee_pending) {
                float4 *nq = reinterpret_cast<float4 *>(ps.nee) + 4 * (size_t)pid;
                if (flags & PF_PEND_SHADOW) nq[0] = make_float4(sh_o.x, sh_o.y, sh_o.z, sh_d.x);
                nq[1] = make_float4(sh_d.y, sh_d.z, 0.0f, __uint_as_float(li)); nq[2] = make_float4(A.r, A.g, A.b, choice_pdf); nq[3] = make_float4(beta.r, beta.g, beta.b, __uint_as_float(sh_medium));
                n_bytes += 48;
            }
        }
    }
    return nee_pending;
}

struct TexMatEval {
    const DeviceScene &s; const TexCtx &c;
    struct Plain {
        const DeviceScene &s; TexCtx c;
        PT_DEV bool bound(const PtMaterial &m, int slot) const { return m.tex[slot] >= 0; }
        PT_DEV RGB spec(const PtMaterial &m, int slot, const float *field) const { return m.tex[slot] >= 0 ? tex_eval(s, m.tex[slot], c) : RGB(field[0], field[1], field[2]); }
        PT_DEV float flt(const PtMaterial &m, int slot, float field) const { return m.tex[slot] >= 0 ? tex_eval(s, m.tex[slot], c).r : field; }
    };
    PT_DEV Plain plain() const { Plain q{s, c}; q.c.dpdx = V3(0.0f, 0.0f, 0.0f); q.c.dpdy = V3(0.0f, 0.0f, 0.0f); q.c.dudx = q.c.dvdx = q.c.dudy = q.c.dvdy = 0.0f; return q; }
    PT_DEV bool bound(const PtMaterial &m, int slot) const { return m.tex[slot] >= 0; }
    PT_DEV RGB spec(const PtMaterial &m, int slot, const float *field) const { return m.tex[slot] >= 0 ? tex_eval(s, m.tex[slot], c) : RGB(field[0], field[1], field[2]); }
    PT_DEV float flt(const PtMaterial &m, int slot, float field) const { return m.tex[slot] >= 0 ? tex_eval(s, m.tex[slot], c).r : field; }
};
PT_DEV RayDiff camera_ray_differentials(const RenderConst &rc, float pfx, float pfy, P2 plens_u, V3 ray_o, V3 ray_d) {
    const V3 pcamera = xf_point(rc.raster_to_camera, V3(pfx, pfy, 0.0f));
    const V3 dxc(rc.dx_camera[0], rc.dx_camera[1], rc.dx_camera[2]), dyc(rc.dy_camera[0], rc.dy_camera[1], rc.dy_camera[2]);
    RayDiff d; d.has = true;
    if (rc.lens_radius > 0.0f) {
        const P2 dk = concentric_sample_disk(plens_u);
        const float lx = dk.x * rc.lens_radius, ly = dk.y * rc.lens_radius;
        const V3 dx = normalize(pcamera + dxc);
        float ft = rc.focal_distance / dx.z;
        V3 pfocus = V3(0.0f, 0.0f, 0.0f) + (dx * ft);
        d.rx_o = V3(lx, ly, 0.0f); d.rx_d = normalize(pfocus - d.rx_o);
        const V3 dy = normalize(pcamera + dyc);
        ft = rc.focal_distance / dy.z;
        pfocus = V3(0.0f, 0.0f, 0.0f) + (dy * ft);
        d.ry_o = V3(lx, ly, 0.0f); d.ry_d = normalize(pfocus - d.ry_o);
    } else {
        d.rx_o = V3(0.0f, 0.0f, 0.0f); d.ry_o = V3(0.0f, 0.0f, 0.0f);
        d.rx_d = normalize(pcamera + dxc); d.ry_d = normalize(pcamera + dyc);
    }
    d.rx_o = xf_point(rc.camera_to_world, d.rx_o); d.ry_o = xf_point(rc.camera_to_world, d.ry_o);
    d.rx_d = xf_vector(rc.camera_to_world, d.rx_d); d.ry_d = xf_vector(rc.camera_to_world, d.ry_d);
    const float sc = rc.inv_sqrt_spp;
    d.rx_o = ray_o + (d.rx_o - ray_o) * sc; d.ry_o = ray_o + (d.ry_o - ray_o) * sc;
    d.rx_d = ray_d + (d.rx_d - ray_d) * sc; d.ry_d = ray_d + (d.ry_d - ray_d) * sc;
    return d;
}
```

### pbrt-rust_amd/csrc/scene_create.hip

```cpp
#include "host_common.h"

#include <memory>

namespace {
PtStatus hlbvh_builder(const std::vector<pth::PrimBound> &pb, uint32_t maxp, std::vector<PtBVHNode> &nodes, std::vector<uint32_t> &ordered, std::string &msg) {
    const char *text = "HLBVH build failed";
    if (!pth::build_hlbvh_gpu(pb, maxp, nodes, ordered, &text)) return PT_OK;
    msg = text;
    return PT_ERR_HIP;
}
struct Uploader {
    pt_scene *sc; int st = PT_OK;
    template <class T> void operator()(const T **field, const T *src, size_t count) { if (!st) st = sc->upload(field, src, count); }
    template <class T> void operator()(const T **field, const std::vector<T> &v) { (*this)(field, v.data(), v.size()); }
};
}

extern "C" {

int pt_scene_create(const PtSceneDesc *d, pt_scene **out) {
    if (!d || !out) return fail(PT_ERR_INVALID_ARG, "null argument");
    std::string msg;
    int st = plan_validate(*d, msg);
    if (st) return fail(st, msg);
    if ((st = ensure_device())) return st;
    ScenePlan plan;
    if ((st = plan_build(*d, PlanOptions{g_shade_specialise, g_test_pool_pad_records}, d->split_method == PT_SPLIT_HLBVH ? AccelBuilder(hlbvh_builder) : AccelBuilder(sah_builder), plan, msg))) return fail(st, msg);
    for (const std::string &w : plan.warnings) fprintf(stderr, "mi355pt: %s\n", w.c_str());

    std::unique_ptr<pt_scene, void (*)(pt_scene *)> owner(new pt_scene(), pt_scene_destroy);
    pt_scene *sc = owner.get();
    DeviceScene &ds = sc->ds;
    sc->device = g_device;
    sc->nodes = std::move(plan.nodes); sc->ordered = std::move(plan.ordered);
    sc->exact_walk_only = plan.exact_walk_only; sc->quad_walk_only = plan.quad_walk_only; sc->pool_big = plan.pool_big;
    std::copy(plan.class_used, plan.class_used + kNumClasses, sc->class_used);
    sc->has_null_material = plan.has_null_material; sc->has_bssrdf = plan.has_bssrdf;
    sc->n_lights = d->n_lights;
    if (d->n_lights) sc->host_lights.assign(d->lights, d->lights + d->n_lights);
    if (d->env_texels) { sc->env_w = d->env_width; sc->env_h = d->env_height; for (int k = 0; k < 3; ++k) sc->env_texel0[k] = d->env_power_lookup[k]; }

    Uploader up{sc};
    up(&ds.wide, plan.wide); ds.root_ref = plan.root_ref; ds.root_ref4 = plan.root_ref4; ds.n_nodes = (uint32_t)sc->nodes.size();
    for (int k = 0; k < 3; ++k) { ds.root_min[k] = sc->nodes[0].bmin[k]; ds.root_max[k] = sc->nodes[0].bmax[k]; }
    up(&ds.instances, plan.instances); ds.n_instances = (uint32_t)plan.instances.size();
    up(&ds.P, d->P, 3 * (size_t)d->n_vertices);
    if (d->N) up(&ds.N, d->N, 3 * (size_t)d->n_vertices);
    if (d->S) up(&ds.S, d->S, 3 * (size_t)d->n_vertices);
    if (d->UV) up(&ds.UV, d->UV, 2 * (size_t)d->n_vertices);
    up(&ds.indices, d->indices, 3 * (size_t)d->n_triangles); ds.n_triangles = d->n_triangles;
    {
        std::vector<uint8_t> fl(d->n_triangles, 0);
        if (d->tri_flags) fl.assign(d->tri_flags, d->tri_flags + d->n_triangles);
        for (auto &f : fl) { if (!d->N) f &= ~PT_TRI_HAS_N; if (!d->S) f &= ~PT_TRI_HAS_S; if (!d->UV) f &= ~PT_TRI_HAS_UV; }
        up(&ds.tri_flags, fl);
    }
    up(&ds.prim_shape, d->prim_shape, d->n_prims); up(&ds.prim_material, d->prim_material, d->n_prims); up(&ds.prim_light, d->prim_light, d->n_prims);
    ds.n_prims = d->n_prims;
    up(&ds.materials, d->materials, d->n_materials); ds.n_materials = d->n_materials;
    if (d->n_media && d->media) {
        up(&ds.media, d->media, d->n_media); ds.n_media = d->n_media;
        for (uint32_t i = 0; i < d->n_media; ++i)
            if (d->media[i].type == PT_MEDIUM_GRID) up(&plan.grid_aux[i].density, d->media[i].density, (size_t)d->media[i].nx * d->media[i].ny * d->media[i].nz);
        up(&ds.grid_aux, plan.grid_aux); ds.has_grid = plan.has_grid ? 1u : 0u;
        if (d->prim_medium_inside && d->prim_medium_outside) { up(&ds.prim_med_in, d->prim_medium_inside, d->n_prims); up(&ds.prim_med_out, d->prim_medium_outside, d->n_prims); }
    }
    ds.has_shells = sc->has_null_material ? 1u : 0u;
    up(&ds.spheres, d->spheres, d->n_spheres); ds.n_spheres = d->n_spheres;
    up(&ds.lights, d->lights, d->n_lights); ds.n_lights = d->n_lights;
    up(&ds.mat_class, plan.mat_class);
    {
        std::vector<DevBssTable> bt(d->n_bssrdf_tables);
        for (uint32_t i = 0; i < d->n_bssrdf_tables; ++i) {
            const PtBSSRDFTable &t = d->bssrdf_tables[i];
            bt[i].n_rho = (int)t.n_rho; bt[i].n_radius = (int)t.n_radius;
            if (!t.rho_samples || !t.radius_samples || !t.profile || !t.rhoeff || !t.profile_cdf) continue;
            up(&bt[i].rho_samples, t.rho_samples, t.n_rho); up(&bt[i].radius_samples, t.radius_samples, t.n_radius);
            up(&bt[i].profile, t.profile, (size_t)t.n_rho * t.n_radius);
            up(&bt[i].rhoeff, t.rhoeff, t.n_rho);
            up(&bt[i].profile_cdf, t.profile_cdf, (size_t)t.n_rho * t.n_radius);
        }
        up(&ds.bss_tables, bt); ds.n_bss_tables = d->n_bssrdf_tables;
    }
    if (d->n_textures) {
        up(&ds.textures, d->textures, d->n_textures); ds.n_textures = d->n_textures;
        up(&ds.tex_prog_offset, plan.tex_prog_offset); up(&ds.tex_prog, plan.tex_prog);
        for (uint32_t i = 0; i < d->n_images; ++i) {
            const PtImage &im = d->images[i];
            if (!im.texels || im.n_levels == 0 || im.n_levels > 16) continue;
            const uint32_t last = im.n_levels - 1;
            up(&plan.images[i].texels, im.texels, plan.images[i].level_offset[last] + (size_t)std::max(1u, im.width >> last) * std::max(1u, im.height >> last) * im.channels);
        }
        up(&ds.images, plan.images);
        if (d->ewa_weight_lut) up(&ds.ewa_lut, d->ewa_weight_lut, 128);
        auto any_mask = [&](const int32_t *a) { if (!a) return false; for (uint32_t i = 0; i < d->n_triangles; ++i) if (a[i] >= 0) return true; return false; };
        if (any_mask(d->tri_alpha)) up(&ds.tri_alpha, d->tri_alpha, d->n_triangles);
        if (any_mask(d->tri_shadow_alpha)) up(&ds.tri_shadow_alpha, d->tri_shadow_alpha, d->n_triangles);
    }
    up(&ds.infinite_lights, plan.infinite_lights); ds.n_infinite = (uint32_t)plan.infinite_lights.size();
    if (d->env_texels) {
        ds.env_w = d->env_width; ds.env_h = d->env_height;
        up(&ds.env_texels, d->env_texels, 3 * (size_t)ds.env_w * ds.env_h);
        up(&ds.env_func, d->env_importance, 4 * (size_t)ds.env_w * ds.env_h); up(&ds.env_cdf, plan.env_cdf); up(&ds.env_func_int, plan.env_func_int);
        up(&ds.env_marg_func, plan.env_func_int); up(&ds.env_marg_cdf, plan.env_marg_cdf); ds.env_marg_int = plan.env_marg_int;
    }
    for (int k = 0; k < 3; ++k) { ds.wb_min[k] = plan.wb_min[k]; ds.wb_max[k] = plan.wb_max[k]; ds.world_center[k] = plan.world_center[k]; }
    ds.world_radius = plan.world_radius;
    const uint32_t *d_ordered = nullptr, *d_last = nullptr;
    up(&d_ordered, plan.packet_refs);
    if (up.st) return up.st;

    const uint32_t n_packets = (uint32_t)plan.packet_refs.size(), n_leaves = (uint32_t)plan.leaf_last.size();
    uint8_t *pool = nullptr; float *area = nullptr; float4 *lrec = nullptr;
    if ((st = sc->dalloc(&pool, plan.pool_bytes))) return st;
    if (plan.pad_bytes && hipMemset(pool, 0, plan.pad_bytes) != hipSuccess) return fail(PT_ERR_HIP, "memset of the pool pad");
    if (hipMemcpy(pool + plan.pad_bytes, plan.quad.data(), plan.quad_bytes - plan.pad_bytes, hipMemcpyHostToDevice) != hipSuccess) return fail(PT_ERR_HIP, "upload of the four-wide records");
    TriPacket *leaf = reinterpret_cast<TriPacket *>(pool + plan.quad_bytes);
    ds.quad = reinterpret_cast<const QuadNode *>(pool); ds.leaf_off = (uint32_t)(plan.quad_bytes / 16); ds.pool_quads = (uint32_t)(plan.pool_bytes / 16);
    if (hipMemset(leaf, 0, ((size_t)n_packets + 2) * sizeof(TriPacket)) != hipSuccess) return fail(PT_ERR_HIP, "memset");
    if ((st = sc->dalloc(&area, std::max<uint32_t>(1, d->n_lights)))) return st;
    if ((st = sc->dalloc(&lrec, 6 * (size_t)std::max<uint32_t>(1, d->n_lights)))) return st;
    up(&d_last, plan.leaf_last);
    if (up.st) return up.st;
    hipLaunchKernelGGL(k_build_packets, dim3((n_packets + 255) / 256), dim3(256), 0, 0, ds, d_ordered, n_packets, leaf);
    ds.leaf = leaf;
    hipLaunchKernelGGL(k_mark_leaf_ends, dim3((n_leaves + 255) / 256), dim3(256), 0, 0, leaf, d_last, n_leaves);
    if (d->n_lights) hipLaunchKernelGGL(k_light_area, dim3((d->n_lights + 255) / 256), dim3(256), 0, 0, ds, area, lrec);
    ds.light_area = area; ds.light_rec = lrec;
    if (hipDeviceSynchronize() != hipSuccess || hipGetLastError() != hipSuccess) return fail(PT_ERR_HIP, "scene preparation kernels failed");
    *out = owner.release();
    return PT_OK;
}

void pt_scene_destroy(pt_scene *sc) {
    if (!sc) return;
    if (sc->device != g_device) bind_device(sc->device);
    for (void *p : sc->allocs) hipFree(p);
    if (sc->slab) hipFree(sc->slab);
    if (sc->qbuf) hipFree(sc->qbuf);
    if (sc->bss_slab) hipFree(sc->bss_slab);
    if (sc->ext_slab) hipFree(sc->ext_slab);
    if (sc->film_rgbw) hipFree(sc->film_rgbw);
    if (sc->tile_list) hipFree(sc->tile_list);
    sc->drop_timings();
    for (auto e : sc->event_pool) hipEventDestroy(e);
    if (sc->stream) hipStreamDestroy(sc->stream);
    delete sc;
}

int pt_scene_bvh_info(const pt_scene *sc, uint32_t *n_nodes, uint32_t *n_prims) {
    if (!sc || !n_nodes || !n_prims) return fail(PT_ERR_INVALID_ARG, "null argument");
    *n_nodes = (uint32_t)sc->nodes.size(); *n_prims = (uint32_t)sc->ordered.size();
    return PT_OK;
}
int pt_scene_bvh_read(const pt_scene *sc, PtBVHNode *nodes, uint32_t *ordered) {
    if (!sc || !nodes || !ordered) return fail(PT_ERR_INVALID_ARG, "null argument");
    std::memcpy(nodes, sc->nodes.data(), sc->nodes.size() * sizeof(PtBVHNode));
    std::memcpy(ordered, sc->ordered.data(), sc->ordered.size() * 4);
    return PT_OK;
}

}
```

### pbrt-rust_amd/csrc/scene_plan.h

```cpp
#pragma once
#include <functional>
#include <string>
#include <vector>
#include "kernels.h"
#include "host_bvh.h"

namespace pth {
using namespace ptd;

uint8_t material_class(const PtMaterial &m, bool specialise, bool untextured);
void dist1d(const std::vector<float> &func, std::vector<float> &cdf, float &func_int);
PrimBound transform_bounds(const float m[16], const float lo[3], const float hi[3]);

struct PlanOptions {
    bool shade_specialise = true;
    uint32_t pool_pad_records = 0;
};
using AccelBuilder = std::function<PtStatus(const std::vector<PrimBound> &prims, uint32_t max_node_prims, std::vector<PtBVHNode> &nodes, std::vector<uint32_t> &ordered, std::string &msg)>;
PtStatus sah_builder(const std::vector<PrimBound> &prims, uint32_t max_node_prims, std::vector<PtBVHNode> &nodes, std::vector<uint32_t> &ordered, std::string &msg);

struct ScenePlan {
    std::vector<PtBVHNode> nodes;
    std::vector<uint32_t> ordered;
    bool exact_walk_only = false, quad_walk_only = false, pool_big = false;
    std::vector<WideNode> wide;
    std::vector<QuadNode> quad;
    uint32_t root_ref = 0, root_ref4 = 0;
    std::vector<uint32_t> packet_refs;
    std::vector<uint32_t> leaf_last;
    std::vector<DevInstance> instances;
    size_t pad_bytes = 0, quad_bytes = 0, pool_bytes = 0;
    std::vector<uint8_t> mat_class;
    bool class_used[kNumClasses] = {true, false, false, false, true, false, false, false, false, false, false};
    bool has_null_material = false, has_bssrdf = false;
    std::vector<uint32_t> infinite_lights;
    std::vector<uint32_t> tex_prog_offset, tex_prog;
    std::vector<DevImage> images;
    std::vector<float> env_cdf, env_func_int, env_marg_cdf; float env_marg_int = 0.0f;
    std::vector<DevGridAux> grid_aux; bool has_grid = false;
    float wb_min[3] = {0, 0, 0}, wb_max[3] = {0, 0, 0}, world_center[3] = {0, 0, 0}, world_radius = 0.0f;
    std::vector<std::string> warnings;
};

PtStatus plan_validate(const PtSceneDesc &d, std::string &msg);
PtStatus plan_build(const PtSceneDesc &d, const PlanOptions &opt, const AccelBuilder &build, ScenePlan &plan, std::string &msg);

}
```

### pbrt-rust_amd/csrc/scene_plan.hip

```cpp
#include <algorithm>
#include <cmath>
#include <cstring>
#include <limits>
#include "scene_plan.h"
#include "dev_bsdf.h"
#include "dev_texture.h"

namespace pth {

uint8_t material_class(const PtMaterial &m, bool specialise, bool untextured) {
    auto textured = [&](int slot) { return m.tex[slot] >= 0; };
    auto black = [](const float c[3]) { return !(c[0] > 0.0f) && !(c[1] > 0.0f) && !(c[2] > 0.0f); };
    switch (m.type) {
    case PT_MAT_MATTE: return 0;
    case PT_MAT_MIRROR: return (uint8_t)kSpecClass;
    case PT_MAT_METAL: return specialise ? (uint8_t)kMetalClass : 1;
    case PT_MAT_SUBSTRATE: return 1;
    case PT_MAT_GLASS:
        if (textured(PT_MP_U_ROUGHNESS) || textured(PT_MP_V_ROUGHNESS)) return 2;
        return (m.u_roughness == 0.0f && m.v_roughness == 0.0f) ? (uint8_t)kSpecClass : 2;
    case PT_MAT_PLASTIC: return specialise ? (uint8_t)kPlasticClass : 2;
    case PT_MAT_UBER: {
        const bool opaque = !textured(PT_MP_OPACITY) && m.opacity[0] >= 1.0f && m.opacity[1] >= 1.0f && m.opacity[2] >= 1.0f;
        const bool no_spec = !textured(PT_MP_KR) && !textured(PT_MP_KT) && black(m.kr) && black(m.kt);
        if (opaque && no_spec) return specialise ? (uint8_t)kPlasticClass : 2;
        return specialise ? (uint8_t)kUberClass : 3;
    }
    case PT_MAT_SUBSURFACE:
        if (specialise && untextured && m.u_roughness == 0.0f && m.v_roughness == 0.0f && !textured(PT_MP_U_ROUGHNESS) && !textured(PT_MP_V_ROUGHNESS)) return (uint8_t)kSssClass;
        return 3;
    default: return 3;
    }
}

void dist1d(const std::vector<float> &func, std::vector<float> &cdf, float &func_int) {
    size_t n = func.size();
    cdf.assign(n + 1, 0.0f);
    for (size_t i = 1; i < n + 1; ++i) cdf[i] = cdf[i - 1] + func[i - 1] / (float)n;
    func_int = cdf[n];
    if (func_int == 0.0f) { for (size_t i = 1; i < n + 1; ++i) cdf[i] = (float)i / (float)n; }
    else { for (size_t i = 1; i < n + 1; ++i) cdf[i] /= func_int; }
}

PrimBound transform_bounds(const float m[16], const float lo[3], const float hi[3]) {
    M4 t; std::memcpy(t.m, m, 64);
    const int corner[8][3] = {{0, 0, 0}, {1, 0, 0}, {0, 1, 0}, {0, 0, 1}, {0, 1, 1}, {1, 1, 0}, {1, 0, 1}, {1, 1, 1}};
    PrimBound out;
    for (int c = 0; c < 8; ++c) {
        V3 p = xf_point(t, V3(corner[c][0] ? hi[0] : lo[0], corner[c][1] ? hi[1] : lo[1], corner[c][2] ? hi[2] : lo[2]));
        const float pc[3] = {p.x, p.y, p.z};
        for (int k = 0; k < 3; ++k) { out.lo[k] = c ? std::fmin(out.lo[k], pc[k]) : pc[k]; out.hi[k] = c ? std::fmax(out.hi[k], pc[k]) : pc[k]; }
    }
    return out;
}

PtStatus sah_builder(const std::vector<PrimBound> &prims, uint32_t max_node_prims, std::vector<PtBVHNode> &nodes, std::vector<uint32_t> &ordered, std::string &) {
    build_sah_bvh(prims, max_node_prims, nodes, ordered);
    return PT_OK;
}

namespace {

PtStatus fail(std::string &msg, PtStatus code, const char *text) { msg = text; return code; }

bool instanced(const PtSceneDesc &d) { return d.n_instances > 0 && d.top_refs && d.n_top > 0; }
int tex_children(const PtTexture &t) {
    return (t.type == PT_TEX_MIX) ? 3 : (t.type == PT_TEX_SCALE || t.type == PT_TEX_CHECKERBOARD2D || t.type == PT_TEX_CHECKERBOARD3D || t.type == PT_TEX_DOTS) ? 2 : 0;
}

PtStatus tex_programs(const PtSceneDesc &d, std::vector<uint32_t> &off, std::vector<uint32_t> &prog, std::string &msg) {
    off.assign(d.n_textures + 1, 0); prog.clear();
    for (uint32_t r = 0; r < d.n_textures; ++r) {
        off[r] = (uint32_t)prog.size();
        struct Fr { int node; int next; };
        std::vector<Fr> st{{(int)r, 0}};
        int depth = 0, max_depth = 0; size_t guard = 0;
        while (!st.empty()) {
            Fr &f = st.back();
            const int nchild = tex_children(d.textures[f.node]);
            if (f.next < nchild) { const int c = d.textures[f.node].child[f.next++]; st.push_back({c, 0}); if (++guard > 4096 || st.size() > 64) return fail(msg, PT_ERR_INVALID_ARG, "texture graph too deep or cyclic"); continue; }
            prog.push_back((uint32_t)f.node);
            depth += 1 - nchild; max_depth = std::max(max_depth, depth + nchild);
            st.pop_back();
        }
        if (max_depth > kTexStack) return fail(msg, PT_ERR_UNSUPPORTED, "texture expression needs a deeper value stack than kTexStack");
    }
    off[d.n_textures] = (uint32_t)prog.size();
    return PT_OK;
}

void prim_bound(const PtSceneDesc &d, uint32_t i, PrimBound &out) {
    const uint32_t idx = d.prim_shape[i] & 0x3fffffffu;
    if ((d.prim_shape[i] >> 30) == PT_SHAPE_SPHERE) {
        const PtSphere &S = d.spheres[idx];
        const float lo[3] = {-S.radius, -S.radius, S.z_min}, hi[3] = {S.radius, S.radius, S.z_max};
        out = transform_bounds(S.object_to_world, lo, hi);
        return;
    }
    const float *a = d.P + 3 * (size_t)d.indices[3 * idx], *b = d.P + 3 * (size_t)d.indices[3 * idx + 1], *c = d.P + 3 * (size_t)d.indices[3 * idx + 2];
    for (int k = 0; k < 3; ++k) { out.lo[k] = std::fmin(std::fmin(a[k], b[k]), c[k]); out.hi[k] = std::fmax(std::fmax(a[k], b[k]), c[k]); }
}

void append_accel(ScenePlan &plan, uint32_t pad_records, const std::vector<PtBVHNode> &nn, const std::vector<uint32_t> &refs, uint32_t &root_ref, uint32_t &root_ref4) {
    std::vector<WideNode> &wide = plan.wide; std::vector<QuadNode> &quad = plan.quad;
    const uint32_t wbase = (uint32_t)wide.size(), pbase = (uint32_t)plan.packet_refs.size();
    std::vector<uint32_t> wide_id(nn.size(), 0);
    uint32_t n_int = 0;
    for (size_t i = 0; i < nn.size(); ++i) { if (nn[i].n_prims == 0) wide_id[i] = wbase + n_int++; else plan.leaf_last.push_back(pbase + nn[i].offset + nn[i].n_prims - 1); }
    auto ref_of = [&](uint32_t i) { return nn[i].n_prims ? (kLeafBit | (pbase + nn[i].offset)) : wide_id[i]; };
    wide.resize(wbase + n_int);
    for (size_t i = 0; i < nn.size(); ++i) {
        if (nn[i].n_prims) continue;
        WideNode &w = wide[wide_id[i]];
        const PtBVHNode &l = nn[i + 1], &r = nn[nn[i].offset];
        w.lmin[0] = l.bmin[0]; w.lmin[1] = l.bmin[1]; w.lmin[2] = l.bmin[2]; w.lmax0 = l.bmax[0];
        w.lmax12[0] = l.bmax[1]; w.lmax12[1] = l.bmax[2]; w.rmin01[0] = r.bmin[0]; w.rmin01[1] = r.bmin[1];
        w.rmin2 = r.bmin[2]; w.rmax[0] = r.bmax[0]; w.rmax[1] = r.bmax[1]; w.rmax[2] = r.bmax[2];
        w.left_ref = ref_of((uint32_t)i + 1); w.right_ref = ref_of(nn[i].offset);
        w.meta = nn[i].axis; w.pad = 0;
    }
    const float inf = std::numeric_limits<float>::infinity();
    std::vector<uint32_t> todo;
    std::vector<uint32_t> quad_id(nn.size(), PT_NONE);
    auto qref_of = [&](uint32_t i) { return nn[i].n_prims ? (kLeafBit | (pbase + nn[i].offset)) : quad_id[i]; };
    const uint32_t qbase = (uint32_t)quad.size();
    if (!nn.empty() && nn[0].n_prims == 0) {
        std::vector<uint32_t> stack{0};
        while (!stack.empty()) {
            const uint32_t i = stack.back(); stack.pop_back();
            quad_id[i] = pad_records + qbase + (uint32_t)todo.size(); todo.push_back(i);
            uint32_t kids[4]; int nk = 0;
            for (uint32_t c : {(uint32_t)i + 1u, (uint32_t)nn[i].offset}) {
                if (nn[c].n_prims) continue;
                kids[nk++] = c + 1u; kids[nk++] = nn[c].offset;
            }
            for (int k = nk - 1; k >= 0; --k) if (nn[kids[k]].n_prims == 0) stack.push_back(kids[k]);
        }
    }
    quad.resize(qbase + todo.size());
    for (size_t t = 0; t < todo.size(); ++t) {
        const uint32_t i = todo[t];
        QuadNode &q = quad[qbase + t];
        for (int a = 0; a < 3; ++a) for (int k = 0; k < 4; ++k) { q.lo[a][k] = inf; q.hi[a][k] = -inf; }
        for (int k = 0; k < 4; ++k) q.ref[k] = PT_NONE;
        q.pad[0] = q.pad[1] = q.pad[2] = 0;
        const uint32_t c2[2] = {i + 1u, (uint32_t)nn[i].offset};
        uint32_t axes[3] = {nn[i].axis, 0u, 0u};
        auto put = [&](int slot, uint32_t n) {
            for (int a = 0; a < 3; ++a) { q.lo[a][slot] = nn[n].bmin[a]; q.hi[a][slot] = nn[n].bmax[a]; }
            q.ref[slot] = qref_of(n);
        };
        for (int side = 0; side < 2; ++side) {
            const uint32_t c = c2[side];
            if (nn[c].n_prims) put(2 * side, c);
            else { axes[1 + side] = nn[c].axis; put(2 * side, c + 1u); put(2 * side + 1, nn[c].offset); }
        }
        q.meta = 0;
        for (uint32_t o = 0; o < 8; ++o) q.meta |= (((o >> axes[0]) & 1u) | (((o >> axes[1]) & 1u) << 1) | (((o >> axes[2]) & 1u) << 2)) << (3u * o);
    }
    root_ref4 = nn.empty() ? 0u : qref_of(0);
    plan.packet_refs.insert(plan.packet_refs.end(), refs.begin(), refs.end());
    root_ref = ref_of(0);
}

}


PtStatus plan_validate(const PtSceneDesc &d, std::string &msg) {
    if (d.n_prims == 0 || !d.prim_shape || !d.prim_material || !d.prim_light) return fail(msg, PT_ERR_INVALID_ARG, "scene has no primitives");
    if (d.n_triangles && (!d.P || !d.indices)) return fail(msg, PT_ERR_INVALID_ARG, "triangle arrays missing");
    if (d.n_spheres && !d.spheres) return fail(msg, PT_ERR_INVALID_ARG, "sphere array missing");
    const bool inst = instanced(d);
    if (d.n_instances && !inst) return fail(msg, PT_ERR_INVALID_ARG, "instances given without top_refs");
    const struct { uint64_t count; const void *array; const char *text; } arrays[] = {
        {d.n_materials, d.materials, "materials array missing"},
        {d.n_lights, d.lights, "lights array missing"},
        {d.n_textures, d.textures, "textures array missing"},
        {d.n_textures ? d.n_images : 0u, d.images, "images array missing"},
        {inst ? d.n_objects : 0u, d.objects, "objects array missing"},
        {inst ? d.n_instances : 0u, d.instances, "instances array missing"},
        {d.n_bssrdf_tables, d.bssrdf_tables, "bssrdf_tables array missing"},
        {d.env_texels ? 1u : 0u, d.env_importance, "env_texels without env_importance"},
        {d.env_texels ? 1u : 0u, (d.env_width && d.env_height) ? d.env_texels : nullptr, "env_texels with a zero env_width or env_height"},
    };
    for (const auto &a : arrays) if (a.count && !a.array) return fail(msg, PT_ERR_INVALID_ARG, a.text);
    for (uint32_t i = 0; i < 3 * d.n_triangles; ++i) if (d.indices[i] >= d.n_vertices) return fail(msg, PT_ERR_INVALID_ARG, "vertex index out of range");
    for (uint32_t i = 0; i < d.n_prims; ++i) {
        uint32_t s = d.prim_shape[i];
        const uint32_t kind = s >> 30, idx = s & 0x3fffffffu;
        if (!((kind == PT_SHAPE_TRIANGLE && idx < d.n_triangles) || (kind == PT_SHAPE_SPHERE && idx < d.n_spheres))) return fail(msg, PT_ERR_INVALID_ARG, "primitive shape reference out of range");
        if (d.prim_material[i] != PT_NONE && d.prim_material[i] >= d.n_materials) return fail(msg, PT_ERR_INVALID_ARG, "material index out of range");
        if (d.prim_light[i] != PT_NONE && d.prim_light[i] >= d.n_lights) return fail(msg, PT_ERR_INVALID_ARG, "light index out of range");
    }
    for (uint32_t i = 0; i < d.n_materials; ++i) {
        const PtMaterial &m = d.materials[i];
        if (m.type != PT_MAT_SUBSURFACE) continue;
        if (!d.bssrdf_tables || m.bssrdf_table >= d.n_bssrdf_tables) return fail(msg, PT_ERR_INVALID_ARG, "subsurface material without a BSSRDF table");
        const PtBSSRDFTable &t = d.bssrdf_tables[m.bssrdf_table];
        if (t.n_rho < 2 || t.n_radius < 2 || !t.rho_samples || !t.radius_samples || !t.profile || !t.rhoeff || !t.profile_cdf) return fail(msg, PT_ERR_INVALID_ARG, "incomplete BSSRDF table");
    }
    for (uint32_t i = 0; i < d.n_textures; ++i) {
        const PtTexture &t = d.textures[i];
        if (t.type > PT_TEX_DOTS) return fail(msg, PT_ERR_UNSUPPORTED, "texture type not implemented");
        for (int k = 0; k < 3; ++k) if (t.child[k] >= (int32_t)d.n_textures) return fail(msg, PT_ERR_INVALID_ARG, "texture child index out of range");
        if (t.type == PT_TEX_IMAGEMAP) {
            if (!d.images || t.image >= d.n_images) return fail(msg, PT_ERR_INVALID_ARG, "image texture without an image");
            const PtImage &im = d.images[t.image];
            auto pow2 = [](uint32_t v) { return v && !(v & (v - 1)); };
            if (!pow2(im.width) || !pow2(im.height) || !im.texels || (im.channels != 1 && im.channels != 3) || im.n_levels == 0 || im.n_levels > 16)
                return fail(msg, PT_ERR_INVALID_ARG, "PtImage must be a power-of-two MIPMap pyramid with 1 or 3 channels");
            if (t.wrap > PT_WRAP_BLACK) return fail(msg, PT_ERR_UNSUPPORTED, "ImageWrap::Clamp is not implemented");
            if (!t.trilinear && !d.ewa_weight_lut) return fail(msg, PT_ERR_INVALID_ARG, "EWA image texture without ewa_weight_lut");
        }
        if (tex_children(t) == 2 && (t.child[0] < 0 || t.child[1] < 0)) return fail(msg, PT_ERR_INVALID_ARG, "texture node needs two children");
        if (t.type == PT_TEX_MIX && (t.child[0] < 0 || t.child[1] < 0 || t.child[2] < 0)) return fail(msg, PT_ERR_INVALID_ARG, "mix texture needs three children");
    }
    for (const int32_t *arr : {d.tri_alpha, d.tri_shadow_alpha})
        if (arr) for (uint32_t i = 0; i < d.n_triangles; ++i) if (arr[i] >= (int32_t)d.n_textures) return fail(msg, PT_ERR_INVALID_ARG, "alpha-mask texture index out of range");
    for (uint32_t i = 0; i < d.n_materials; ++i) {
        const PtMaterial &m = d.materials[i];
        if (m.type > PT_MAT_DISNEY) return fail(msg, PT_ERR_INVALID_ARG, "unknown material type");
        if (m.type == PT_MAT_DISNEY) {
            const bool thin = m.disney_thin != 0;
            const float dw = (1.0f - m.disney[PT_DS_METALLIC]) * (1.0f - m.disney[PT_DS_SPECTRANS]);
            int n = 1 + (m.disney[PT_DS_CLEARCOAT] > 0.0f) + (m.disney[PT_DS_SPECTRANS] > 0.0f) + (thin ? 1 : 0);
            if (dw > 0.0f) n += (thin ? 2 : 1) + 1 + (m.disney[PT_DS_SHEEN] > 0.0f);
            if (n > 5) return fail(msg, PT_ERR_UNSUPPORTED, "disney material with more than 5 BxDFs");
            if (disney_has_bssrdf(m) && d.n_textures && m.tex[PT_MP_KD] >= 0) return fail(msg, PT_ERR_UNSUPPORTED, "disney: a textured color together with scatterdistance");
            if (disney_has_bssrdf(m) && (m.disney_scatter[0] <= 0.0f || m.disney_scatter[1] <= 0.0f || m.disney_scatter[2] <= 0.0f)) return fail(msg, PT_ERR_INVALID_ARG, "disney: scatterdistance must be positive in every channel");
        }
        if (m.type == PT_MAT_MIX) {
            auto lobes = [](const PtMaterial &q) { switch (q.type) { case PT_MAT_GLASS: return 2; case PT_MAT_PLASTIC: return 2; case PT_MAT_UBER: return 5; case PT_MAT_TRANSLUCENT: return 4; case PT_MAT_DISNEY: return 5; default: return 1; } };
            int total = 0;
            for (int k = 0; k < 2; ++k) {
                if (m.mix[k] >= d.n_materials) return fail(msg, PT_ERR_INVALID_ARG, "mix material index out of range");
                const PtMaterial &q = d.materials[m.mix[k]];
                if (q.type == PT_MAT_MIX || q.type == PT_MAT_SUBSURFACE || disney_has_bssrdf(q)) return fail(msg, PT_ERR_UNSUPPORTED, "mix of mix / subsurface materials");
                total += lobes(q);
            }
            if (total > 5) return fail(msg, PT_ERR_UNSUPPORTED, "mix material with more than 5 BxDFs");
        }
        for (int k = 0; k < 16; ++k) {
            if (d.n_textures == 0 && m.tex[k] > 0) return fail(msg, PT_ERR_INVALID_ARG, "material references a texture but the scene has none");
            if (d.n_textures && m.tex[k] >= (int32_t)d.n_textures) return fail(msg, PT_ERR_INVALID_ARG, "material texture index out of range");
        }
    }
    for (uint32_t i = 0; i < d.n_lights; ++i) {
        const PtLight &L = d.lights[i];
        if (L.type == PT_LIGHT_DIFFUSE_AREA && L.prim >= d.n_prims) return fail(msg, PT_ERR_INVALID_ARG, "area light primitive out of range");
        if (L.type == PT_LIGHT_INFINITE && !d.env_texels) return fail(msg, PT_ERR_INVALID_ARG, "infinite light without env_texels");
    }
    if (d.split_method > PT_SPLIT_HLBVH) return fail(msg, PT_ERR_INVALID_ARG, "unknown split_method");
    const uint32_t n_top = inst ? d.n_top : d.n_prims;
    if (inst) {
        for (uint32_t o = 0; o < d.n_objects; ++o)
            if (d.objects[o].n_prims == 0 || (uint64_t)d.objects[o].first_prim + d.objects[o].n_prims > d.n_prims) return fail(msg, PT_ERR_INVALID_ARG, "object primitive range out of bounds");
        for (uint32_t i = 0; i < d.n_instances; ++i) if (d.instances[i].object >= d.n_objects) return fail(msg, PT_ERR_INVALID_ARG, "instance object index out of range");
        for (uint32_t i = 0; i < n_top; ++i) {
            uint32_t r = d.top_refs[i];
            if ((r & PT_TOP_INSTANCE) ? ((r & ~PT_TOP_INSTANCE) >= d.n_instances) : (r >= d.n_prims)) return fail(msg, PT_ERR_INVALID_ARG, "top_refs entry out of range");
        }
    }
    if (d.nodes && d.n_nodes && d.ordered_prims) {
        for (uint32_t i = 0; i < n_top; ++i) if (d.ordered_prims[i] >= n_top) return fail(msg, PT_ERR_INVALID_ARG, "ordered_prims entry out of range");
        for (uint32_t i = 0; i < d.n_nodes; ++i) {
            const PtBVHNode &n = d.nodes[i];
            bool ok = n.n_prims ? ((uint64_t)n.offset + n.n_prims <= n_top) : (n.offset < d.n_nodes && n.offset > i + 1 && n.axis < 3);
            if (!ok) return fail(msg, PT_ERR_INVALID_ARG, "malformed BVH node");
        }
    }
    if (d.n_media && d.media) {
        for (uint32_t i = 0; i < d.n_media; ++i) {
            const PtMedium &m = d.media[i];
            if (m.type > PT_MEDIUM_GRID) return fail(msg, PT_ERR_INVALID_ARG, "unknown medium type");
            if (m.type != PT_MEDIUM_GRID) continue;
            const size_t nvox = (size_t)m.nx * m.ny * m.nz;
            if (!m.density || nvox == 0 || nvox > ((size_t)1 << 31)) return fail(msg, PT_ERR_INVALID_ARG, "grid medium without a density grid");
            size_t k = 0;
            while (k < nvox && !(m.density[k] > 0.0f)) ++k;
            if (k == nvox) return fail(msg, PT_ERR_INVALID_ARG, "grid medium with no positive density");
        }
        if (d.prim_medium_inside && d.prim_medium_outside)
            for (uint32_t i = 0; i < d.n_prims; ++i)
                if ((d.prim_medium_inside[i] != PT_NONE && d.prim_medium_inside[i] >= d.n_media) || (d.prim_medium_outside[i] != PT_NONE && d.prim_medium_outside[i] >= d.n_media))
                    return fail(msg, PT_ERR_INVALID_ARG, "primitive medium index out of range");
    }
    std::vector<uint32_t> off, prog;
    return tex_programs(d, off, prog, msg);
}

PtStatus plan_build(const PtSceneDesc &d, const PlanOptions &opt, const AccelBuilder &build, ScenePlan &plan, std::string &msg) {
    PtStatus st;
    const bool inst = instanced(d);
    const uint32_t n_top = inst ? d.n_top : d.n_prims;
    const uint32_t maxp = d.max_node_prims ? d.max_node_prims : 4;
    struct ObjAccel { std::vector<PtBVHNode> nodes; std::vector<uint32_t> ordered; };
    std::vector<ObjAccel> obj(inst ? d.n_objects : 0);
    for (uint32_t o = 0; o < obj.size(); ++o) {
        const PtObject &O = d.objects[o];
        if (O.n_prims == 1) continue;
        std::vector<PrimBound> pb(O.n_prims);
        for (uint32_t i = 0; i < O.n_prims; ++i) prim_bound(d, O.first_prim + i, pb[i]);
        if ((st = build(pb, maxp, obj[o].nodes, obj[o].ordered, msg))) return st;
        for (auto &e : obj[o].ordered) e += O.first_prim;
    }
    auto top_ref = [&](uint32_t pos) { return inst ? d.top_refs[pos] : pos; };
    if (d.nodes && d.n_nodes && d.ordered_prims) {
        plan.nodes.assign(d.nodes, d.nodes + d.n_nodes);
        plan.ordered.assign(d.ordered_prims, d.ordered_prims + n_top);
        for (uint32_t i = 0; i < d.n_nodes && !plan.exact_walk_only; ++i) {
            const PtBVHNode &n = plan.nodes[i];
            if (n.n_prims) continue;
            for (uint32_t c : {i + 1u, (uint32_t)n.offset}) for (int k = 0; k < 3; ++k)
                if (!(plan.nodes[c].bmin[k] >= n.bmin[k] && plan.nodes[c].bmax[k] <= n.bmax[k])) plan.exact_walk_only = true;
        }
    } else {
        std::vector<PrimBound> pb(n_top);
        for (uint32_t i = 0; i < n_top; ++i) {
            const uint32_t r = top_ref(i);
            if (!(r & PT_TOP_INSTANCE)) { prim_bound(d, r, pb[i]); continue; }
            const PtInstance &I = d.instances[r & ~PT_TOP_INSTANCE];
            const PtObject &O = d.objects[I.object];
            PrimBound inner;
            if (O.n_prims == 1) prim_bound(d, O.first_prim, inner);
            else for (int k = 0; k < 3; ++k) { inner.lo[k] = obj[I.object].nodes[0].bmin[k]; inner.hi[k] = obj[I.object].nodes[0].bmax[k]; }
            pb[i] = transform_bounds(I.instance_to_world, inner.lo, inner.hi);
        }
        if ((st = build(pb, maxp, plan.nodes, plan.ordered, msg))) return st;
    }
    {
        std::vector<uint32_t> top_order(n_top);
        for (uint32_t i = 0; i < n_top; ++i) top_order[i] = top_ref(plan.ordered[i]);
        append_accel(plan, opt.pool_pad_records, plan.nodes, top_order, plan.root_ref, plan.root_ref4);
    }
    std::vector<uint32_t> obj_root(obj.size(), 0), obj_root4(obj.size(), 0);
    for (size_t o = 0; o < obj.size(); ++o) {
        if (d.objects[o].n_prims == 1) {
            obj_root[o] = obj_root4[o] = kLeafBit | (uint32_t)plan.packet_refs.size();
            plan.leaf_last.push_back((uint32_t)plan.packet_refs.size());
            plan.packet_refs.push_back(d.objects[o].first_prim);
        } else append_accel(plan, opt.pool_pad_records, obj[o].nodes, obj[o].ordered, obj_root[o], obj_root4[o]);
    }
    plan.instances.resize(inst ? d.n_instances : 0);
    for (size_t i = 0; i < plan.instances.size(); ++i) {
        const PtInstance &I = d.instances[i]; DevInstance &D = plan.instances[i];
        std::memcpy(D.world_to_instance, I.world_to_instance, 64); std::memcpy(D.instance_to_world, I.instance_to_world, 64);
        D.single = d.objects[I.object].n_prims == 1; D.root_ref = obj_root[I.object]; D.root_ref4 = obj_root4[I.object];
        for (int k = 0; k < 3; ++k) { D.root_min[k] = D.single ? 0.0f : obj[I.object].nodes[0].bmin[k]; D.root_max[k] = D.single ? 0.0f : obj[I.object].nodes[0].bmax[k]; }
        bool ident = true;
        for (int r = 0; r < 4; ++r) for (int c = 0; c < 4; ++c) ident = ident && I.instance_to_world[4 * r + c] == ((r == c) ? 1.0f : 0.0f);
        D.identity = ident;
    }
    if (plan.quad.size() + opt.pool_pad_records >= ((size_t)1 << 28) || plan.packet_refs.size() >= ((size_t)1 << 31) - 2) return fail(msg, PT_ERR_UNSUPPORTED, "scene exceeds 2^28 four-wide BVH records / 2^31 packets");
    if (plan.wide.size() > (size_t)kRefMask || plan.packet_refs.size() > (size_t)kRefMask) { plan.quad_walk_only = true; plan.wide.clear(); plan.wide.shrink_to_fit(); }
    if (plan.exact_walk_only && plan.quad_walk_only) return fail(msg, PT_ERR_UNSUPPORTED, "adopted BVH whose child boxes do not nest inside their parents' (needs the two-wide walk) in a scene beyond 2^25 records / packets (has the four-wide walk only)");
    if (plan.exact_walk_only) plan.warnings.push_back("warning: the adopted BVH's child boxes do not nest inside their parents'; this scene is walked two-wide, box by box (slower than the four-wide production walk)");
    if (plan.wide.empty()) plan.wide.resize(1);
    if (plan.quad.empty()) plan.quad.resize(1);
    plan.pad_bytes = (size_t)opt.pool_pad_records * sizeof(QuadNode);
    plan.quad_bytes = plan.pad_bytes + plan.quad.size() * sizeof(QuadNode);
    plan.pool_bytes = plan.quad_bytes + (plan.packet_refs.size() + 2) * sizeof(TriPacket);
    if (plan.pool_bytes / 16 >= (size_t)0xfffffff0u) return fail(msg, PT_ERR_UNSUPPORTED, "scene exceeds 64 GB of traversal records + packets");
    plan.pool_big = plan.pool_bytes >= (size_t)0xE0000000u;
    plan.mat_class.assign(std::max<uint32_t>(1, d.n_materials), 0);
    for (uint32_t i = 0; i < d.n_materials; ++i) {
        plan.mat_class[i] = material_class(d.materials[i], opt.shade_specialise, d.n_textures == 0); plan.class_used[plan.mat_class[i]] = true;
        if (d.materials[i].type == PT_MAT_SUBSURFACE || disney_has_bssrdf(d.materials[i])) plan.has_bssrdf = true;
    }
    for (uint32_t i = 0; i < d.n_prims; ++i) if (d.prim_material[i] == PT_NONE) plan.has_null_material = true;
    for (uint32_t i = 0; i < d.n_lights; ++i) if (d.lights[i].type == PT_LIGHT_INFINITE) plan.infinite_lights.push_back(i);
    if (d.n_textures) {
        if ((st = tex_programs(d, plan.tex_prog_offset, plan.tex_prog, msg))) return st;
        plan.images.resize(d.n_images);
        for (uint32_t i = 0; i < d.n_images; ++i) {
            const PtImage &im = d.images[i]; DevImage &out = plan.images[i];
            out.width = im.width; out.height = im.height; out.n_levels = im.n_levels; out.channels = im.channels;
            if (!im.texels || im.n_levels == 0 || im.n_levels > 16) continue;
            size_t o = 0;
            for (uint32_t l = 0; l < im.n_levels; ++l) { out.level_offset[l] = (uint32_t)o; o += (size_t)std::max(1u, im.width >> l) * std::max(1u, im.height >> l) * im.channels; }
        }
    }
    if (d.n_media && d.media) {
        plan.grid_aux.assign(d.n_media, DevGridAux{nullptr, 0.0f, 0.0f});
        for (uint32_t i = 0; i < d.n_media; ++i) {
            const PtMedium &m = d.media[i];
            if (m.type != PT_MEDIUM_GRID) continue;
            for (int k = 1; k < 3; ++k) if (m.sigma_a[k] + m.sigma_s[k] != m.sigma_a[0] + m.sigma_s[0]) { plan.warnings.push_back("GridDensityMedium requires spectrally uniform attenuation coefficient (medium " + std::to_string(i) + ": using channel 0, as grid.rs:46-52 does)"); break; }
            const size_t nvox = (size_t)m.nx * m.ny * m.nz;
            float maxd = 0.0f;
            for (size_t k = 0; k < nvox; ++k) maxd = std::fmax(maxd, m.density[k]);
            plan.grid_aux[i].sigma_t = m.sigma_a[0] + m.sigma_s[0]; plan.grid_aux[i].inv_max_density = 1.0f / maxd;
            plan.has_grid = true;
        }
        plan.class_used[kMediumClass] = true;
    }
    if (d.env_texels) {
        const size_t nu = 2 * (size_t)d.env_width, nv = 2 * (size_t)d.env_height;
        plan.env_cdf.resize(nv * (nu + 1)); plan.env_func_int.resize(nv);
        std::vector<float> row, c;
        for (size_t v = 0; v < nv; ++v) {
            row.assign(d.env_importance + v * nu, d.env_importance + (v + 1) * nu);
            dist1d(row, c, plan.env_func_int[v]);
            std::copy(c.begin(), c.end(), plan.env_cdf.begin() + v * (nu + 1));
        }
        dist1d(plan.env_func_int, plan.env_marg_cdf, plan.env_marg_int);
    }
    bool inside = true;
    for (int k = 0; k < 3; ++k) {
        plan.wb_min[k] = plan.nodes[0].bmin[k]; plan.wb_max[k] = plan.nodes[0].bmax[k];
        plan.world_center[k] = (plan.wb_min[k] + plan.wb_max[k]) * (1.0f / 2.0f);
        inside = inside && plan.world_center[k] >= plan.wb_min[k] && plan.world_center[k] <= plan.wb_max[k];
    }
    const float dx = plan.wb_max[0] - plan.world_center[0], dy = plan.wb_max[1] - plan.world_center[1], dz = plan.wb_max[2] - plan.world_center[2];
    plan.world_radius = inside ? std::sqrt(dx * dx + dy * dy + dz * dz) : 0.0f;
    return PT_OK;
}

}
```

Measured before the change: 1940.

## Pack light type into records and route env lookups through constant memory

```diff
diff --git a/pbrt-rust_amd/csrc/dev_light.h b/pbrt-rust_amd/csrc/dev_light.h
--- a/pbrt-rust_amd/csrc/dev_light.h
+++ b/pbrt-rust_amd/csrc/dev_light.h
@@ -58,6 +58,10 @@
     d = t - o;
 }
 
+typedef const __attribute__((address_space(4))) EnvUniform *EnvBlock;
+typedef const __attribute__((address_space(4))) float *ConstFloats;
+PT_DEV EnvBlock env_block(const DeviceScene &s) { return (EnvBlock)s.env_u; }
+
 PT_DEV RGB env_lookup(const DeviceScene &s, P2 st) {
     int w = (int)s.env_w, h = (int)s.env_h;
     float sf = st.x * (float)w - 0.5f, tf = st.y * (float)h - 0.5f;
@@ -68,6 +72,15 @@
         int64_t r = v % n; if (r < 0) r += n;
         return (int)r;
     };
+    if (w == 1 && h == 1) {
+        const EnvBlock e = env_block(s);
+        const RGB c(e->texel0[0], e->texel0[1], e->texel0[2]);
+        RGB tmp1 = c * (ds * dt);
+        RGB tmp2 = c * (ds * (1.0f - dt));
+        RGB tmp3 = c * ((1.0f - ds) * dt);
+        RGB tmp4 = c * ((1.0f - ds) * (1.0f - dt));
+        return tmp4 + tmp3 + tmp2 + tmp1;
+    }
     const int sa = wrap(s0, w), sb = wrap(s0 + 1, w), ta = wrap(t0, h), tb = wrap(t0 + 1, h);
     auto texel = [&](int si, int ti) -> RGB {
         const float *p = s.env_texels + 3 * ((size_t)ti * w + si);
@@ -80,41 +93,80 @@
     return tmp4 + tmp3 + tmp2 + tmp1;
 }
 
-PT_DEV bool light_is_delta(const PtLight &L) { return L.type == PT_LIGHT_DISTANT || L.type == PT_LIGHT_POINT || L.type == PT_LIGHT_SPOT; }
+PT_DEV uint32_t light_head(const DeviceScene &s, uint32_t li) { return __float_as_uint(s.light_rec[6 * (size_t)li].w); }
+PT_DEV uint32_t head_type(uint32_t head) { return (head >> kLrecTypeShift) & kLrecTypeMask; }
+PT_DEV bool head_is_delta(uint32_t head) { return (head & kLrecDelta) != 0u; }
 
 PT_DEV RGB area_l(const PtLight &L, V3 n, V3 w) {
     if (L.two_sided || dot(n, w) > 0.0f) return RGB(L.L[0], L.L[1], L.L[2]);
     return RGB(0.0f);
 }
-struct LightTri { V3 p0, p1, p2, n_sample, n_pdf; uint32_t fl, tri; float area, inv_area; RGB Lemit; bool two_sided, degenerate; };
+struct LightTri { V3 p0, p1, p2, n_sample, n_pdf; uint32_t fl, tri, head; float area, inv_area; RGB Lemit; bool two_sided, degenerate; };
 PT_DEV bool load_light_tri(const DeviceScene &s, uint32_t li, LightTri &t, bool for_pdf) {
     const float4 *r = s.light_rec + 6 * (size_t)li;
     const float4 q0 = r[0], q1 = r[1], q2 = r[2];
     t.p0 = V3(q0.x, q0.y, q0.z); t.p1 = V3(q1.x, q1.y, q1.z); t.p2 = V3(q2.x, q2.y, q2.z);
     const uint32_t bits = __float_as_uint(q0.w);
-    t.fl = bits & 0xffu; t.degenerate = (bits & 0x200u) != 0u; t.tri = __float_as_uint(q1.w); t.area = q2.w;
+    t.head = bits; t.fl = bits & 0xffu; t.degenerate = (bits & kLrecDegenerate) != 0u; t.tri = __float_as_uint(q1.w); t.area = q2.w;
     if (for_pdf) { const float4 q5 = r[5]; t.n_pdf = V3(q5.x, q5.y, q5.z); }
     else {
         const float4 q3 = r[3], q4 = r[4];
         t.Lemit = RGB(q3.x, q3.y, q3.z); t.two_sided = __float_as_uint(q3.w) != 0u;
         t.n_sample = V3(q4.x, q4.y, q4.z); t.inv_area = q4.w;
     }
-    return (bits & 0x100u) != 0u;
+    return (bits & kLrecValid) != 0u;
+}
+PT_DEV RGB area_l_rec(const DeviceScene &s, uint32_t li, V3 n, V3 w) {
+    const float4 q3 = s.light_rec[6 * (size_t)li + 3];
+    return (__float_as_uint(q3.w) != 0u || dot(n, w) > 0.0f) ? RGB(q3.x, q3.y, q3.z) : RGB(0.0f);
 }
 PT_DEV RGB area_l(const LightTri &t, V3 n, V3 w) { return (t.two_sided || dot(n, w) > 0.0f) ? t.Lemit : RGB(0.0f); }
 PT_DEV M4 ldm4(const float *p) { M4 m; for (int i = 0; i < 16; ++i) m.m[i] = p[i]; return m; }
-
-PT_DEV RGB light_le(const DeviceScene &s, const PtLight &L, V3 ray_d) {
-    if (L.type != PT_LIGHT_INFINITE) return RGB(0.0f);
-    V3 w = normalize(xf_vector(ldm4(L.world_to_light), ray_d));
+PT_DEV M4 ldm4(ConstFloats p) { M4 m; for (int i = 0; i < 16; ++i) m.m[i] = p[i]; return m; }
+
+PT_DEV M4 env_world_to_light(const DeviceScene &s, uint32_t li) { const EnvBlock e = env_block(s); return li == e->light ? ldm4(e->world_to_light) : ldm4(s.lights[li].world_to_light); }
+PT_DEV M4 env_light_to_world(const DeviceScene &s, uint32_t li) { const EnvBlock e = env_block(s); return li == e->light ? ldm4(e->light_to_world) : ldm4(s.lights[li].light_to_world); }
+PT_DEV RGB light_le_infinite(const DeviceScene &s, uint32_t li, V3 ray_d) {
+    V3 w = normalize(xf_vector(env_world_to_light(s, li), ray_d));
     P2 st(spherical_phi(w) * kInv2Pi, spherical_theta(w) * kInvPi);
     return env_lookup(s, st);
 }
+PT_DEV RGB light_le(const DeviceScene &s, uint32_t li, V3 ray_d) {
+    if (head_type(light_head(s, li)) != PT_LIGHT_INFINITE) return RGB(0.0f);
+    return light_le_infinite(s, li, ray_d);
+}
+
+PT_DEV float dist2_sample_continuous(float c0, float c1, float c2, float f0, float f1, float func_int, float u, float &pdf, int &off) {
+    int first = 0, len = 3;
+    while (len > 0) {
+        const int half = len >> 1, middle = first + half;
+        const float cm = middle == 0 ? c0 : middle == 1 ? c1 : c2;
+        if (cm <= u) { first = middle + 1; len -= half + 1; }
+        else len = half;
+    }
+    const int r = first - 1;
+    off = r < 0 ? 0 : (r > 1 ? 1 : r);
+    const float co = off == 0 ? c0 : c1, cn = off == 0 ? c1 : c2;
+    float du = u - co;
+    float diff = cn - co;
+    if (diff > 0.0f) du /= diff;
+    pdf = (func_int > 0.0f) ? (off == 0 ? f0 : f1) / func_int : 0.0f;
+    return ((float)off + du) / 2.0f;
+}
 
 PT_DEV P2 env_sample_continuous(const DeviceScene &s, P2 u, float &pdf) {
     int nu = 2 * (int)s.env_w, nv = 2 * (int)s.env_h;
+    float pdf1, pdf0; int v, dummy;
+    if (s.env_w == 1 && s.env_h == 1) {
+        const EnvUniform __attribute__((address_space(4))) &e = *env_block(s);
+        float d1 = dist2_sample_continuous(e.marg_cdf[0], e.marg_cdf[1], e.marg_cdf[2], e.row_int[0], e.row_int[1], e.marg_int, u.y, pdf1, v);
+        const bool v0 = v == 0;
+        float d0 = dist2_sample_continuous(v0 ? e.row_cdf[0][0] : e.row_cdf[1][0], v0 ? e.row_cdf[0][1] : e.row_cdf[1][1], v0 ? e.row_cdf[0][2] : e.row_cdf[1][2],
+                                           v0 ? e.row_func[0][0] : e.row_func[1][0], v0 ? e.row_func[0][1] : e.row_func[1][1], v0 ? e.row_int[0] : e.row_int[1], u.x, pdf0, dummy);
+        pdf = pdf0 * pdf1;
+        return P2(d0, d1);
+    }
     Dist1D marg{s.env_marg_func, s.env_marg_cdf, s.env_marg_int, nv};
-    float pdf1, pdf0; int v, dummy;
     float d1 = dist_sample_continuous(marg, u.y, pdf1, v);
     Dist1D cond{s.env_func + (size_t)v * nu, s.env_cdf + (size_t)v * (nu + 1), s.env_func_int[v], nu};
     float d0 = dist_sample_continuous(cond, u.x, pdf0, dummy);
@@ -125,6 +177,7 @@
     int nu = 2 * (int)s.env_w, nv = 2 * (int)s.env_h;
     uint32_t iu = f2u32_sat(p.x * (float)nu); if (iu > (uint32_t)(nu - 1)) iu = nu - 1;
     uint32_t iv = f2u32_sat(p.y * (float)nv); if (iv > (uint32_t)(nv - 1)) iv = nv - 1;
+    if (s.env_w == 1 && s.env_h == 1) { const EnvBlock e = env_block(s); return (iv == 0 ? (iu == 0 ? e->row_func[0][0] : e->row_func[0][1]) : (iu == 0 ? e->row_func[1][0] : e->row_func[1][1])) / e->marg_int; }
     return s.env_func[(size_t)iv * nu + iu] / s.env_marg_int;
 }
 
@@ -173,11 +226,13 @@
     return it;
 }
 
-template <bool SPH> PT_DEV RGB light_sample_li(const DeviceScene &s, uint32_t li, const IData &ref, P2 u, V3 &wi, float &pdf, IData &p1) {
+template <bool SPH> PT_DEV RGB light_sample_li_rec(const DeviceScene &s, uint32_t li, const IData &ref, P2 u, V3 &wi, float &pdf, IData &p1, uint32_t &head) {
     p1.p = V3(); p1.p_error = V3(); p1.n = V3();
     {
         LightTri t;
-        if (load_light_tri(s, li, t, false)) {
+        const bool is_tri = load_light_tri(s, li, t, false);
+        head = t.head;
+        if (is_tri) {
             const float su0 = sqrtf(u.x);
             const float b0 = 1.0f - su0, b1 = u.y * su0;
             IData it;
@@ -205,9 +260,10 @@
             return area_l(t, it.n, -wi);
         }
     }
-    const PtLight &L = s.lights[li];
-    switch (L.type) {
+    switch (head_type(head)) {
     case PT_LIGHT_DIFFUSE_AREA: {
+        if (!SPH) { pdf = 0.0f; return RGB(0.0f); }
+        const PtLight &L = s.lights[li];
         if (SPH && (s.prim_shape[L.prim] >> 30) == PT_SHAPE_SPHERE && s.spheres[s.prim_shape[L.prim] & 0x3fffffffu].kind == PT_QUADRIC_DISK) {
             const PtSphere &S = s.spheres[s.prim_shape[L.prim] & 0x3fffffffu];
             const P2 pd = concentric_sample_disk(u);
@@ -239,18 +295,21 @@
         pdf = 0.0f; return RGB(0.0f);
     }
     case PT_LIGHT_DISTANT: {
+        const PtLight &L = s.lights[li];
         V3 wl(L.dir[0], L.dir[1], L.dir[2]);
         wi = wl; pdf = 1.0f;
         p1.p = ref.p + wl * (2.0f * s.world_radius);
         return RGB(L.L[0], L.L[1], L.L[2]);
     }
     case PT_LIGHT_POINT: {
+        const PtLight &L = s.lights[li];
         V3 pl(L.pos[0], L.pos[1], L.pos[2]);
         wi = normalize(pl - ref.p); pdf = 1.0f;
         p1.p = pl;
         return RGB(L.L[0], L.L[1], L.L[2]) / distance_squared(pl, ref.p);
     }
     case PT_LIGHT_SPOT: {
+        const PtLight &L = s.lights[li];
         V3 pl(L.pos[0], L.pos[1], L.pos[2]);
         wi = normalize(pl - ref.p); pdf = 1.0f;
         p1.p = pl;
@@ -270,7 +329,7 @@
         dm_sincosf(theta, sin_t, cos_t);
         dm_sincosf(phi, sin_p, cos_p);
         V3 v(sin_t * cos_p, sin_t * sin_p, cos_t);
-        wi = xf_vector(ldm4(L.light_to_world), v);
+        wi = xf_vector(env_light_to_world(s, li), v);
         pdf = map_pdf / (2.0f * kPi * kPi * sin_t);
         if (sin_t == 0.0f) pdf = 0.0f;
         p1.p = ref.p + wi * (2.0f * s.world_radius);
@@ -279,11 +338,18 @@
     default: pdf = 0.0f; return RGB(0.0f);
     }
 }
+template <bool SPH> PT_DEV RGB light_sample_li(const DeviceScene &s, uint32_t li, const IData &ref, P2 u, V3 &wi, float &pdf, IData &p1) {
+    uint32_t head;
+    return light_sample_li_rec<SPH>(s, li, ref, u, wi, pdf, p1, head);
+}
 
 template <bool SPH> PT_DEV float light_pdf_li(const DeviceScene &s, uint32_t li, const IData &ref, V3 wi) {
+    uint32_t type;
     {
         LightTri t;
-        if (load_light_tri(s, li, t, true)) {
+        const bool is_tri = load_light_tri(s, li, t, true);
+        type = head_type(t.head);
+        if (is_tri) {
             V3 o; spawn_ray(ref, wi, o);
             float th, b0, b1, b2;
             if (!tri_hit_params(t.p0, t.p1, t.p2, o, wi, PT_INF, th, b0, b1, b2)) return 0.0f;
@@ -295,8 +361,16 @@
             return pdf;
         }
     }
+    if (type == PT_LIGHT_INFINITE) {
+        V3 w = xf_vector(env_world_to_light(s, li), wi);
+        float theta = spherical_theta(w), phi = spherical_phi(w);
+        float sin_t = dm_sinf(theta);
+        if (sin_t == 0.0f) return 0.0f;
+        return env_pdf(s, P2(phi * kInv2Pi, theta * kInvPi)) / (2.0f * kPi * kPi * sin_t);
+    }
+    if (!SPH || type != PT_LIGHT_DIFFUSE_AREA) return 0.0f;
     const PtLight &L = s.lights[li];
-    if (SPH && L.type == PT_LIGHT_DIFFUSE_AREA && (s.prim_shape[L.prim] >> 30) == PT_SHAPE_SPHERE && s.spheres[s.prim_shape[L.prim] & 0x3fffffffu].kind == PT_QUADRIC_DISK) {
+    if (SPH && (s.prim_shape[L.prim] >> 30) == PT_SHAPE_SPHERE && s.spheres[s.prim_shape[L.prim] & 0x3fffffffu].kind == PT_QUADRIC_DISK) {
         const PtSphere &S = s.spheres[s.prim_shape[L.prim] & 0x3fffffffu];
         V3 o; spawn_ray(ref, wi, o);
         SurfaceInteraction il;
@@ -305,7 +379,7 @@
         if (__builtin_isinf(pdf)) pdf = 0.0f;
         return pdf;
     }
-    if (SPH && L.type == PT_LIGHT_DIFFUSE_AREA && (s.prim_shape[L.prim] >> 30) == PT_SHAPE_SPHERE) {
+    if (SPH && (s.prim_shape[L.prim] >> 30) == PT_SHAPE_SPHERE) {
         const PtSphere &S = s.spheres[s.prim_shape[L.prim] & 0x3fffffffu];
         const V3 pcenter = xf_point(ldm4g(S.object_to_world), V3(0.0f, 0.0f, 0.0f));
         const V3 porigin = offset_ray_origin(ref.p, ref.p_error, ref.n, pcenter - ref.p);
@@ -320,14 +394,6 @@
         const float sin_thetamax2 = S.radius * S.radius / distance_squared(ref.p, pcenter);
         const float cos_thetamax = sqrtf(maxf(1.0f - sin_thetamax2, 0.0f));
         return 1.0f / (2.0f * kPi * (1.0f - cos_thetamax));
-    }
-    if (L.type == PT_LIGHT_DIFFUSE_AREA) return 0.0f;
-    if (L.type == PT_LIGHT_INFINITE) {
-        V3 w = xf_vector(ldm4(L.world_to_light), wi);
-        float theta = spherical_theta(w), phi = spherical_phi(w);
-        float sin_t = dm_sinf(theta);
-        if (sin_t == 0.0f) return 0.0f;
-        return env_pdf(s, P2(phi * kInv2Pi, theta * kInvPi)) / (2.0f * kPi * kPi * sin_t);
     }
     return 0.0f;
 }
diff --git a/pbrt-rust_amd/csrc/dev_scene.h b/pbrt-rust_amd/csrc/dev_scene.h
--- a/pbrt-rust_amd/csrc/dev_scene.h
+++ b/pbrt-rust_amd/csrc/dev_scene.h
@@ -45,6 +45,18 @@
 struct DevBssTable { int n_rho, n_radius; const float *rho_samples, *radius_samples, *profile, *rhoeff, *profile_cdf; };
 
 struct DevImage { uint32_t width, height, n_levels, channels; const float *texels; uint32_t level_offset[16]; };
+
+struct EnvUniform {
+    uint32_t light;
+    float world_to_light[16], light_to_world[16];
+    float texel0[3];
+    float marg_cdf[3], marg_int, row_int[2];
+    float row_cdf[2][3], row_func[2][2];
+};
+constexpr uint32_t kLrecValid = 0x100u, kLrecDegenerate = 0x200u, kLrecDelta = 0x400u, kLrecTypeShift = 12, kLrecTypeMask = 15u;
+PT_HD uint32_t light_rec_head(uint32_t type) {
+    return ((type & kLrecTypeMask) << kLrecTypeShift) | ((type == PT_LIGHT_DISTANT || type == PT_LIGHT_POINT || type == PT_LIGHT_SPOT) ? kLrecDelta : 0u);
+}
 
 struct DeviceScene {
     const WideNode *wide; uint32_t n_nodes;
@@ -65,9 +77,11 @@
     const DevBssTable *bss_tables; uint32_t n_bss_tables;
     const PtMedium *media; uint32_t n_media;
     uint32_t has_shells;
-    const DevGridAux *grid_aux; uint32_t has_grid;
+    const DevGridAux *grid_aux; uint32_t has_grid; uint32_t n_textures;
     const uint32_t *prim_med_in; const uint32_t *prim_med_out;
-    const PtTexture *textures; uint32_t n_textures; const uint32_t *tex_prog_offset; const uint32_t *tex_prog;
+    const PtTexture *textures;
+    const EnvUniform *env_u;
+    const uint32_t *tex_prog_offset; const uint32_t *tex_prog;
     const DevImage *images; const float *ewa_lut;
     const int32_t *tri_alpha; const int32_t *tri_shadow_alpha;
     uint32_t env_w, env_h; const float *env_texels;
diff --git a/pbrt-rust_amd/csrc/kern_decl.h b/pbrt-rust_amd/csrc/kern_decl.h
--- a/pbrt-rust_amd/csrc/kern_decl.h
+++ b/pbrt-rust_amd/csrc/kern_decl.h
@@ -10,7 +10,7 @@
 __global__ void k_shade_medium(DeviceScene s, RenderConst rc, SobolTables tabs, LightGrid grid, PathSoA ps, ShadeJob job);
 __global__ void k_build_packets(DeviceScene s, const uint32_t *ordered, uint32_t n_refs, TriPacket *out);
 __global__ void k_mark_leaf_ends(TriPacket *leaf, const uint32_t *last_index, uint32_t n);
-__global__ void k_light_area(DeviceScene s, float *area, float4 *rec);
+__global__ void k_light_area(DeviceScene s, const uint32_t *head, float *area, float4 *rec);
 template <int NQ, int CAP> __global__ void k_route(DeviceScene s, const uint32_t *queue, const uint32_t *count_ptr, PathSoA ps, uint32_t *class_count, RouteJob rj);
 __global__ void k_generate(RenderConst rc, SobolTables tabs, PathSoA ps, uint32_t *q_ext, uint32_t *q_ext_count, DevCounters *counters);
 __global__ void k_film(RenderConst rc, PathSoA ps, const float *filter_table, float *film_rgbw, DevCounters *counters);
diff --git a/pbrt-rust_amd/csrc/kern_misc.h b/pbrt-rust_amd/csrc/kern_misc.h
--- a/pbrt-rust_amd/csrc/kern_misc.h
+++ b/pbrt-rust_amd/csrc/kern_misc.h
@@ -38,12 +38,12 @@
     if (i < n) leaf[last_index[i]].flags |= TP_LAST;
 }
 
-__global__ void k_light_area(DeviceScene s, float *area, float4 *rec) {
+__global__ void k_light_area(DeviceScene s, const uint32_t *head, float *area, float4 *rec) {
     uint32_t i = blockIdx.x * blockDim.x + threadIdx.x;
     if (i >= s.n_lights) return;
     float a = 0.0f;
     const PtLight &L = s.lights[i];
-    float4 r0 = make_float4(0.0f, 0.0f, 0.0f, 0.0f), r1 = r0, r2 = r0, r4 = r0, r5 = r0;
+    float4 r0 = make_float4(0.0f, 0.0f, 0.0f, __uint_as_float(head[i])), r1 = make_float4(0.0f, 0.0f, 0.0f, 0.0f), r2 = r1, r4 = r1, r5 = r1;
     if (L.type == PT_LIGHT_DIFFUSE_AREA) {
         uint32_t shape = s.prim_shape[L.prim];
         if ((shape >> 30) == PT_SHAPE_TRIANGLE) {
@@ -60,7 +60,7 @@
             V3 dpdu, dpdv;
             const bool degenerate = !tri_partials(p0, p1, p2, uv, dpdu, dpdv);
             r4 = make_float4(ns.x, ns.y, ns.z, 1.0f / a); r5 = make_float4(np.x, np.y, np.z, 0.0f);
-            r0 = make_float4(p0.x, p0.y, p0.z, __uint_as_float(fl | 0x100u | (degenerate ? 0x200u : 0u)));
+            r0 = make_float4(p0.x, p0.y, p0.z, __uint_as_float(fl | kLrecValid | (degenerate ? kLrecDegenerate : 0u) | head[i]));
             r1 = make_float4(p1.x, p1.y, p1.z, __uint_as_float(tri)); r2 = make_float4(p2.x, p2.y, p2.z, a);
         } else {
             const PtSphere &S = s.spheres[shape & 0x3fffffffu];
diff --git a/pbrt-rust_amd/csrc/kern_shade_common.h b/pbrt-rust_amd/csrc/kern_shade_common.h
--- a/pbrt-rust_amd/csrc/kern_shade_common.h
+++ b/pbrt-rust_amd/csrc/kern_shade_common.h
@@ -50,7 +50,6 @@
     if (flags & PF_PEND_MIS) {
         const float4 *mq = reinterpret_cast<const float4 *>(ps.mis) + 4 * (size_t)pid;
         const float4 m0 = EARLY ? e0 : mq[0], m1 = EARLY ? e1 : mq[1], m2 = EARLY ? e2 : mq[2], m3 = EARLY ? e3 : mq[3];
-        const PtLight &Lt = s.lights[li];
         V3 wi(m0.w, m1.x, m1.y);
         RGB lrad(0.0f);
         const uint32_t mp = __float_as_uint(m2.x);
@@ -58,9 +57,9 @@
             if (s.prim_light[mp] == li) {
                 SurfaceInteraction lsi;
                 fill_hit<SPH>(s, mp, PT_NONE, V3(m0.x, m0.y, m0.z), wi, m2.y, m2.z, m2.w, lsi);
-                lrad = area_l(Lt, lsi.n, -wi);
-            }
-        } else { PT_T(2); lrad = light_le(s, Lt, wi); PT_T(1); }
+                lrad = area_l_rec(s, li, lsi.n, -wi);
+            }
+        } else { PT_T(2); lrad = light_le(s, li, wi); PT_T(1); }
         RGB Tr(1.0f);
         bool tr_done = false;
         if (VOL) {
@@ -197,7 +196,7 @@
 }
 
 PT_DEV void add_escaped_le(const DeviceScene &s, V3 rd, RGB beta, RGB &L) {
-    for (uint32_t k = 0; k < s.n_infinite; ++k) L = L + light_le(s, s.lights[s.infinite_lights[k]], rd) * beta;
+    for (uint32_t k = 0; k < s.n_infinite; ++k) L = L + light_le_infinite(s, s.infinite_lights[k], rd) * beta;
 }
 
 PT_DEV void hist_init(uint32_t *s_hist) { if (threadIdx.x < 16) s_hist[threadIdx.x] = 0; }
@@ -229,9 +228,10 @@
             RGB A(0.0f); V3 sh_o(0.0f, 0.0f, 0.0f), sh_d(0.0f, 0.0f, 0.0f);
             uint32_t sh_medium = PT_NONE;
             PT_T(6);
-            RGB Li = light_sample_li<SPH>(s, li, it, ulight, wi, lightpdf, p1);
+            uint32_t lhead;
+            RGB Li = light_sample_li_rec<SPH>(s, li, it, ulight, wi, lightpdf, p1, lhead);
             PT_T(7);
-            const bool delta = light_is_delta(s.lights[li]);
+            const bool delta = head_is_delta(lhead);
             if (lightpdf > 0.0f && !Li.is_black()) {
                 RGB f = bsdf.f_pdf(si.wo, wi, bf, scattpdf);
                 if (!MEDIUM) f = f * abs_dot(wi, si.sh_n);
diff --git a/pbrt-rust_amd/csrc/scene_create.hip b/pbrt-rust_amd/csrc/scene_create.hip
--- a/pbrt-rust_amd/csrc/scene_create.hip
+++ b/pbrt-rust_amd/csrc/scene_create.hip
@@ -98,6 +98,7 @@
         if (any_mask(d->tri_shadow_alpha)) up(&ds.tri_shadow_alpha, d->tri_shadow_alpha, d->n_triangles);
     }
     up(&ds.infinite_lights, plan.infinite_lights); ds.n_infinite = (uint32_t)plan.infinite_lights.size();
+    up(&ds.env_u, &plan.env_u, 1);
     if (d->env_texels) {
         ds.env_w = d->env_width; ds.env_h = d->env_height;
         up(&ds.env_texels, d->env_texels, 3 * (size_t)ds.env_w * ds.env_h);
@@ -106,8 +107,8 @@
     }
     for (int k = 0; k < 3; ++k) { ds.wb_min[k] = plan.wb_min[k]; ds.wb_max[k] = plan.wb_max[k]; ds.world_center[k] = plan.world_center[k]; }
     ds.world_radius = plan.world_radius;
-    const uint32_t *d_ordered = nullptr, *d_last = nullptr;
-    up(&d_ordered, plan.packet_refs);
+    const uint32_t *d_ordered = nullptr, *d_last = nullptr, *d_head = nullptr;
+    up(&d_ordered, plan.packet_refs); up(&d_head, plan.light_head);
     if (up.st) return up.st;
 
     const uint32_t n_packets = (uint32_t)plan.packet_refs.size(), n_leaves = (uint32_t)plan.leaf_last.size();
@@ -125,7 +126,7 @@
     hipLaunchKernelGGL(k_build_packets, dim3((n_packets + 255) / 256), dim3(256), 0, 0, ds, d_ordered, n_packets, leaf);
     ds.leaf = leaf;
     hipLaunchKernelGGL(k_mark_leaf_ends, dim3((n_leaves + 255) / 256), dim3(256), 0, 0, leaf, d_last, n_leaves);
-    if (d->n_lights) hipLaunchKernelGGL(k_light_area, dim3((d->n_lights + 255) / 256), dim3(256), 0, 0, ds, area, lrec);
+    if (d->n_lights) hipLaunchKernelGGL(k_light_area, dim3((d->n_lights + 255) / 256), dim3(256), 0, 0, ds, d_head, area, lrec);
     ds.light_area = area; ds.light_rec = lrec;
     if (hipDeviceSynchronize() != hipSuccess || hipGetLastError() != hipSuccess) return fail(PT_ERR_HIP, "scene preparation kernels failed");
     *out = owner.release();
diff --git a/pbrt-rust_amd/csrc/scene_plan.h b/pbrt-rust_amd/csrc/scene_plan.h
--- a/pbrt-rust_amd/csrc/scene_plan.h
+++ b/pbrt-rust_amd/csrc/scene_plan.h
@@ -37,6 +37,8 @@
     std::vector<uint32_t> tex_prog_offset, tex_prog;
     std::vector<DevImage> images;
     std::vector<float> env_cdf, env_func_int, env_marg_cdf; float env_marg_int = 0.0f;
+    EnvUniform env_u;
+    std::vector<uint32_t> light_head;
     std::vector<DevGridAux> grid_aux; bool has_grid = false;
     float wb_min[3] = {0, 0, 0}, wb_max[3] = {0, 0, 0}, world_center[3] = {0, 0, 0}, world_radius = 0.0f;
     std::vector<std::string> warnings;
diff --git a/pbrt-rust_amd/csrc/scene_plan.hip b/pbrt-rust_amd/csrc/scene_plan.hip
--- a/pbrt-rust_amd/csrc/scene_plan.hip
+++ b/pbrt-rust_amd/csrc/scene_plan.hip
@@ -369,6 +369,8 @@
     }
     for (uint32_t i = 0; i < d.n_prims; ++i) if (d.prim_material[i] == PT_NONE) plan.has_null_material = true;
     for (uint32_t i = 0; i < d.n_lights; ++i) if (d.lights[i].type == PT_LIGHT_INFINITE) plan.infinite_lights.push_back(i);
+    plan.light_head.assign(std::max<uint32_t>(1, d.n_lights), 0u);
+    for (uint32_t i = 0; i < d.n_lights; ++i) plan.light_head[i] = light_rec_head(d.lights[i].type);
     if (d.n_textures) {
         if ((st = tex_programs(d, plan.tex_prog_offset, plan.tex_prog, msg))) return st;
         plan.images.resize(d.n_images);
@@ -405,6 +407,23 @@
         }
         dist1d(plan.env_func_int, plan.env_marg_cdf, plan.env_marg_int);
     }
+    std::memset(&plan.env_u, 0, sizeof plan.env_u);
+    plan.env_u.light = PT_NONE;
+    if (!plan.infinite_lights.empty()) {
+        const PtLight &L = d.lights[plan.infinite_lights[0]];
+        plan.env_u.light = plan.infinite_lights[0];
+        std::copy(L.world_to_light, L.world_to_light + 16, plan.env_u.world_to_light); std::copy(L.light_to_world, L.light_to_world + 16, plan.env_u.light_to_world);
+    }
+    if (d.env_texels && d.env_width == 1 && d.env_height == 1) {
+        EnvUniform &e = plan.env_u;
+        std::copy(d.env_texels, d.env_texels + 3, e.texel0);
+        std::copy(plan.env_marg_cdf.begin(), plan.env_marg_cdf.begin() + 3, e.marg_cdf); e.marg_int = plan.env_marg_int;
+        for (int v = 0; v < 2; ++v) {
+            e.row_int[v] = plan.env_func_int[v];
+            std::copy(plan.env_cdf.begin() + 3 * v, plan.env_cdf.begin() + 3 * v + 3, e.row_cdf[v]);
+            std::copy(d.env_importance + 2 * v, d.env_importance + 2 * v + 2, e.row_func[v]);
+        }
+    }
     bool inside = true;
     for (int k = 0; k < 3; ++k) {
         plan.wb_min[k] = plan.nodes[0].bmin[k]; plan.wb_max[k] = plan.nodes[0].bmax[k];
```

New measurement: 1993, median of 6. 1.03x the previous value.
